# bnbowman/pbccs

Hardware: AMD Instinct MI355X
Metric: CCS ZMWs/sec (and GCUPS) at 1/2/4/8 MI355X vs host-CPU ccs (higher is better)
Workload: dtype f64

## Files before the change

pbccs_amd/csrc/arrow_kernels.hpp:

```cpp
#pragma once

#include <hip/hip_runtime.h>

#include "arrow_device.hpp"

namespace pbccs {

struct ScoreWork {
    int nWork = 0;
    const int* zmw = nullptr;
    const int* nMut = nullptr;
    const long long* mutBase = nullptr;
    const long long* deltaBase = nullptr;
    const long long* waveStart = nullptr;
    const long long* mutStart = nullptr;
    const long long* posStart = nullptr;
    const int* codes = nullptr;
    double* delta = nullptr;
    int* edgeList = nullptr;
    int* edgeCount = nullptr;
    int edgeCap = 0;
    int readLo = 0;
    int readHi = 1 << 30;
    const long long* sel = nullptr;
    const long long* selBase = nullptr;
    const int* nSel = nullptr;
    const double* dev = nullptr;
    int* amb = nullptr;
};

constexpr int kCkptMaxK = 32;
constexpr unsigned long long kCkptBadGeometry = 1ull << 62;
struct CkptWork {
    const int2* pairs = nullptr;
    const long long* taskStart = nullptr;
    int nPairs = 0;
    long long nTasks = 0;
    unsigned long long* counter = nullptr;
    double* slots = nullptr;
    long long slotCap = 0;
    int nSlots = 0;
    unsigned long long* need = nullptr;
};

struct ScoreScratch {
    double* pool = nullptr;
    unsigned long long* top = nullptr;
    unsigned long long cap = 0;
    int* overflow = nullptr;
};

struct FillScratch {
    double* val = nullptr;
    int2* range = nullptr;
    int* off = nullptr;
    double* ls = nullptr;
    double* pre = nullptr;
    int* usedA = nullptr;
    int* usedB = nullptr;
    long long capSlots = 0;
    int capCols = 0;
    long long* trace = nullptr;
};

struct CoopFill {
    int* usedA = nullptr;
    int* usedB = nullptr;
    int* maxH = nullptr;
    int hcap = 0;
    int readWords = 0;
    int tplWords = 0;
    size_t groupBytes = 0;
    bool prio = false;
    bool chainExit = true;
    bool scan = false;
    double devScale = 1.0;
    int rows = 1;
    double thrMargin = 0x1p-50;
    int regrowSlackDiv = 16;
    unsigned long long* valBump = nullptr;
    long long valLimit = 0;
    long long* rValA = nullptr;
    long long* rValB = nullptr;
    long long* rValCap = nullptr;
    double* colScratch = nullptr;
    int gRows = 0;
    long long* trace = nullptr;
    unsigned long long* work = nullptr;
};
enum FillWork : int {
    kFillWorkCells = 0, kFillWorkTallAbort, kFillWorkRegrow, kFillWorkOverflow, kFillWorkSteps, kFillWorkIssues,
    kFillWorkReads, kFillWorkPasses, kFillWorkSlots
};
size_t coop_group_bytes(int hcap, int readWords, int tplWords);
constexpr int kNarrowGroupLanes = 16;
constexpr int kTallRowsPerLane = 2;
void launch_fill_coop(int G, const DevBatch& B, const CoopFill& F, const int* reads, int n, hipStream_t s);

void launch_fill(const DevBatch& B, const FillScratch& F, const int* reads, int n, hipStream_t s);
void launch_compact(const DevBatch& B, const FillScratch& F, const int* reads, int n, hipStream_t s);
void launch_suffix(const DevBatch& B, const int* reads, int n, hipStream_t s, bool withPrefix = false);
void launch_enumerate(const DevBatch& B, const int* zmws, int n, const long long* mutBase, const long long* posBase,
                      int* codes, int* posOff, hipStream_t s);
void launch_score(const DevBatch& B, const ScoreWork& W, long long nWaves, const ScoreScratch& scratch, hipStream_t s,
                  const CkptWork* ck = nullptr);
void launch_alive(const DevBatch& B, const ScoreWork& W, long long nMut, double fastThr, int readHi,
                  unsigned char* alive, hipStream_t s);
void launch_sel_ranges(const ScoreWork& W, const long long* sel, const long long* count, long long* selBase,
                       int* nSel, hipStream_t s);
void launch_reduce(const DevBatch& B, const ScoreWork& W, long long nMut, double fastThr, double* score,
                   unsigned char* fav, hipStream_t s);
void launch_best_subset(int nWork, const long long* selBase, const int* nSel, const int* code, const double* score,
                        int sep, int ldsCap, int* rank, hipStream_t s);
void launch_qv(const DevBatch& B, const ScoreWork& W, long long nPos, const long long* posBase, const int* posOff,
               const double* score, const long long* qvBase, int* qv, hipStream_t s);

}
```

pbccs_amd/csrc/engine.hip:

```cpp
#include "engine.hpp"

#include <hipcub/hipcub.hpp>

#include <algorithm>
#include <mutex>
#include <climits>
#include <cmath>
#include <cstdio>
#include <cstdlib>
#include <cstring>
#include <numeric>
#include <stdexcept>
#include <chrono>
#include <unordered_set>

namespace pbccs {

#define PBCCS_HIP(x)                                                         \
    do {                                                                     \
        hipError_t e_ = (x);                                                 \
        if (e_ != hipSuccess) throw DeviceError(hipGetErrorString(e_));      \
    } while (0)

const char* const kKernelNames[kKernelKinds] = {"k_fill",       "k_suffix",      "k_enumerate", "k_score",
                                                 "k_reduce",     "k_qv",          "k_best_subset", "k_compact",
                                                 "k_fill_tall",  "k_qfill_grp",   "k_qfill_coop", "k_qfill",
                                                 "k_qscore_mid", "k_qscore_multi"};

namespace {

constexpr int kFillBandHeight = 28;
constexpr double kFillScratchBudget = 24.0 * (1ull << 30);
constexpr int kCoopNarrowRows = 64;
constexpr int kCoopTallRows = 1024;
constexpr size_t kCoopLdsBytes = 60 * 1024;
constexpr int kHybridRows = 1536;
constexpr size_t kHeadroomMargin = 24ull << 30;
constexpr long long kTallFirstDiv = 25;
constexpr int kCkptDefaultK = 8;
constexpr int kCkptDefaultMinLen = 4000;
constexpr int kCkptSlotsMax = 2048;
constexpr long long kCkptSlotBytes = 1ll << 30;
int env_int(const char* name, int dflt)
{
    const char* e = std::getenv(name);
    return e ? std::atoi(e) : dflt;
}
constexpr long long kPhasedMinTasks = 1 << 21;
constexpr size_t kInitialScratch = 1 << 20;
constexpr int kMaxCopySegs = 8;

template <class T>
void upload(DevVec<T>& d, const std::vector<T>& h, hipStream_t s)
{
    d.reserve(std::max<size_t>(h.size(), 1), false);
    if (!h.empty()) PBCCS_HIP(hipMemcpyAsync(d.ptr, h.data(), h.size() * sizeof(T), hipMemcpyHostToDevice, s));
}

void d2h(void* dst, const void* src, size_t bytes, hipStream_t s)
{
    static const bool drain = env_int("PBCCS_D2H_DRAIN", 1) != 0;
    if (!bytes) return;
    if (drain) PBCCS_HIP(hipStreamSynchronize(s));
    PBCCS_HIP(hipMemcpyAsync(dst, src, bytes, hipMemcpyDeviceToHost, s));
}

template <class T>
void download(std::vector<T>& h, const DevVec<T>& d, size_t n, hipStream_t s)
{
    h.resize(n);
    d2h(h.data(), d.ptr, n * sizeof(T), s);
}

struct CopySeg {
    const unsigned int* src;
    unsigned int* dst;
    unsigned long long words;
};
struct CopySegs {
    CopySeg s[kMaxCopySegs];
};
__global__ void __launch_bounds__(256) k_copy_segs(CopySegs g)
{
    const CopySeg q = g.s[blockIdx.y];
    for (unsigned long long k = (unsigned long long)blockIdx.x * 256 + threadIdx.x; k < q.words;
         k += (unsigned long long)gridDim.x * 256)
        q.dst[k] = q.src[k];
}

struct Xfer {
    void* dev;
    void* host;
    size_t bytes;
};

size_t stage_layout(const std::vector<Xfer>& items, std::vector<size_t>* off)
{
    size_t top = 0;
    off->clear();
    for (const Xfer& x : items) {
        if (x.bytes % 4) throw DeviceError("packed transfer of a size not a multiple of 4 bytes");
        off->push_back(top);
        top += (x.bytes + 15) & ~(size_t)15;
    }
    return top;
}

void launch_copy_segs(const std::vector<CopySeg>& segs, hipStream_t s)
{
    for (size_t b = 0; b < segs.size(); b += kMaxCopySegs) {
        CopySegs g{};
        const int n = (int)std::min(segs.size() - b, (size_t)kMaxCopySegs);
        unsigned long long most = 0;
        for (int k = 0; k < n; ++k) {
            g.s[k] = segs[b + k];
            most = std::max(most, segs[b + k].words);
        }
        if (!most) continue;
        const unsigned gx = (unsigned)std::min<unsigned long long>((most + 255) / 256, 1024);
        hipLaunchKernelGGL(k_copy_segs, dim3(gx, n), dim3(256), 0, s, g);
        PBCCS_HIP(hipGetLastError());
    }
}

void download_packed(const std::vector<Xfer>& items, DevVec<unsigned char>& stage, std::vector<unsigned char>& host,
                     hipStream_t s)
{
    std::vector<size_t> off;
    const size_t top = stage_layout(items, &off);
    if (!top) return;
    stage.reserve(top, false);
    std::vector<CopySeg> segs;
    for (size_t k = 0; k < items.size(); ++k)
        if (items[k].bytes)
            segs.push_back({static_cast<const unsigned int*>(items[k].dev),
                            reinterpret_cast<unsigned int*>(stage.ptr + off[k]), items[k].bytes / 4});
    launch_copy_segs(segs, s);
    host.resize(top);
    d2h(host.data(), stage.ptr, top, s);
    PBCCS_HIP(hipStreamSynchronize(s));
    for (size_t k = 0; k < items.size(); ++k)
        if (items[k].bytes) std::memcpy(items[k].host, host.data() + off[k], items[k].bytes);
}

void upload_packed(const std::vector<Xfer>& items, DevVec<unsigned char>& stage, std::vector<unsigned char>& host,
                   hipStream_t s)
{
    std::vector<size_t> off;
    const size_t top = stage_layout(items, &off);
    if (!top) return;
    stage.reserve(top, false);
    host.resize(top);
    std::vector<CopySeg> segs;
    for (size_t k = 0; k < items.size(); ++k) {
        if (!items[k].bytes) continue;
        std::memcpy(host.data() + off[k], items[k].host, items[k].bytes);
        segs.push_back({reinterpret_cast<const unsigned int*>(stage.ptr + off[k]),
                        static_cast<unsigned int*>(items[k].dev), items[k].bytes / 4});
    }
    PBCCS_HIP(hipMemcpyAsync(stage.ptr, host.data(), top, hipMemcpyHostToDevice, s));
    launch_copy_segs(segs, s);
}

template <class T>
Xfer xfer_dl(std::vector<T>& h, const DevVec<T>& d, size_t n)
{
    h.resize(n);
    return Xfer{d.ptr, h.data(), n * sizeof(T)};
}

template <class T>
Xfer xfer_ul(DevVec<T>& d, const std::vector<T>& h)
{
    d.reserve(std::max<size_t>(h.size(), 1), false);
    return Xfer{d.ptr, const_cast<T*>(h.data()), h.size() * sizeof(T)};
}

}

static bool va_used_before(void* va)
{
    static std::mutex mu;
    static std::vector<void*> used;
    std::lock_guard<std::mutex> lk(mu);
    if (std::find(used.begin(), used.end(), va) != used.end()) return true;
    used.push_back(va);
    return false;
}

void VmPool::try_reserve(size_t n)
{
    if (!vmm_ || n <= cap) return;
    map_to(n, true);
}

void VmPool::reserve(size_t n, bool keep)
{
    if (n <= cap) return;
    if (!tried_ && allowVmm) {
        tried_ = true;
        void* va = nullptr;
        static const bool dbgVa = env_int("PBCCS_DBG_VA", 0) != 0;
        for (int attempt = 0;; ++attempt) {
            vmm_ = hipMemAddressReserve(&va, kVaBytes, 0, nullptr, 0) == hipSuccess && va != nullptr;
            if (!vmm_) {
                (void)hipGetLastError();
                break;
            }
            if (dbgVa) std::fprintf(stderr, "[vmpool %p] reserve va=%p (%zu parked)\n", (void*)this, va, parkedVas_.size());
            if (!va_used_before(va)) break;
            reusedVas_ += 1;
            parkedVas_.push_back(va);
            if (attempt == 64) throw DeviceError("band pool: no address range this pool has not mapped before");
        }
        if (vmm_) ptr = static_cast<double*>(va);
    }
    if (!vmm_) {
        fallback_.reserve(n, keep);
        ptr = fallback_.ptr;
        cap = fallback_.cap;
        return;
    }
    map_to(n, false);
}

void VmPool::map_to(size_t n, bool soft)
{
    size_t want = n * sizeof(double);
    if (want > kVaBytes) {
        if (!soft) throw DeviceError("band pool exceeds its address reservation");
        want = kVaBytes;
    }
    size_t capBytes = kVaBytes;
    if (const char* e = std::getenv("PBCCS_POOL_CAP_MB")) {
        const long long mb = std::atoll(e);
        if (mb > 0) capBytes = std::min(kVaBytes, (size_t)mb << 20);
    }
    if (want > capBytes) {
        if (!soft)
            throw DeviceOom("band pool capped at " + std::to_string(capBytes >> 20) + " MB (PBCCS_POOL_CAP_MB), needs " +
                            std::to_string(want >> 20) + " MB");
        want = capBytes;
    }
    int dev = 0;
    PBCCS_HIP(hipGetDevice(&dev));
    hipMemAllocationProp prop = {};
    prop.type = hipMemAllocationTypePinned;
    prop.location.type = hipMemLocationTypeDevice;
    prop.location.id = dev;
    hipMemAccessDesc desc = {};
    desc.location = prop.location;
    desc.flags = hipMemAccessFlagsProtReadWrite;
    while (mappedBytes_ < want) {
        const size_t bytes = std::min(std::min(kChunkBytes, capBytes), kVaBytes - mappedBytes_);
        if (mappedBytes_ + bytes > capBytes) break;
        hipMemGenericAllocationHandle_t h;
        if (hipMemCreate(&h, bytes, &prop, 0) != hipSuccess) {
            (void)hipGetLastError();
            if (soft) break;
            size_t fr = 0, tot = 0;
            (void)hipMemGetInfo(&fr, &tot);
            throw DeviceOom("hipMemCreate failed (device memory): band pool at " + std::to_string(mappedBytes_ >> 30) +
                              " GB, needs " + std::to_string(want >> 30) + " GB, " + std::to_string(fr >> 20) +
                              " MB free");
        }
        char* at = reinterpret_cast<char*>(ptr) + mappedBytes_;
        if (hipMemMap(at, bytes, 0, h, 0) != hipSuccess) {
            (void)hipMemRelease(h);
            throw DeviceError("hipMemMap failed");
        }
        if (hipMemSetAccess(at, bytes, &desc, 1) != hipSuccess) {
            (void)hipMemUnmap(at, bytes);
            (void)hipMemRelease(h);
            throw DeviceError("hipMemSetAccess failed");
        }
        handles_.push_back(h);
        sizes_.push_back(bytes);
        mappedBytes_ += bytes;
    }
    cap = mappedBytes_ / sizeof(double);
    if (!soft && mappedBytes_ < want)
        throw DeviceOom("band pool capped at " + std::to_string(capBytes >> 20) + " MB (PBCCS_POOL_CAP_MB), needs " +
                        std::to_string(want >> 20) + " MB");
}

void VmPool::unmap_all(hipStream_t s)
{
    if (!vmm_) {
        if (s) (void)hipStreamSynchronize(s);
        fallback_.release();
        ptr = nullptr;
        cap = 0;
        return;
    }
    if (s) (void)hipStreamSynchronize(s);
    else (void)hipDeviceSynchronize();
    static const bool dbgVa = env_int("PBCCS_DBG_VA", 0) != 0;
    if (dbgVa) std::fprintf(stderr, "[vmpool %p] unmap_all va=%p mapped=%zu MB\n", (void*)this, (void*)ptr, mappedBytes_ >> 20);
    size_t off = 0;
    for (size_t k = 0; k < handles_.size(); ++k) {
        (void)hipMemUnmap(reinterpret_cast<char*>(ptr) + off, sizes_[k]);
        (void)hipMemRelease(handles_[k]);
        off += sizes_[k];
    }
    handles_.clear();
    sizes_.clear();
    mappedBytes_ = 0;
    cap = 0;
    (void)hipMemAddressFree(ptr, kVaBytes);
    ptr = nullptr;
    tried_ = false;
    vmm_ = false;
}

VmPool::~VmPool()
{
    for (void* va : parkedVas_) (void)hipMemAddressFree(va, kVaBytes);
    if (!vmm_) return;
    (void)hipDeviceSynchronize();
    size_t off = 0;
    for (size_t k = 0; k < handles_.size(); ++k) {
        (void)hipMemUnmap(reinterpret_cast<char*>(ptr) + off, sizes_[k]);
        (void)hipMemRelease(handles_[k]);
        off += sizes_[k];
    }
    (void)hipMemAddressFree(ptr, kVaBytes);
}

void ckpt_policy(int* K, int* minLen)
{
    *K = std::min(kCkptMaxK, std::max(0, env_int("PBCCS_CKPT_K", kCkptDefaultK)));
    *minLen = std::max(0, env_int("PBCCS_CKPT_MIN_LEN", kCkptDefaultMinLen));
}

Workspace::~Workspace()
{
    if (stream) (void)hipStreamSynchronize(stream);
    if (stream2) (void)hipStreamSynchronize(stream2);
    for (hipEvent_t e : eventPool) (void)hipEventDestroy(e);
    if (evFork) (void)hipEventDestroy(evFork);
    if (evJoin) (void)hipEventDestroy(evJoin);
    if (stream2) (void)hipStreamDestroy(stream2);
    if (stream) (void)hipStreamDestroy(stream);
}

size_t Workspace::TrimRetired()
{
    size_t b = 0;
    auto t = [&](auto& v) { b += v.trim(); };
    t(hDesc);
    t(selBase); t(nSel); t(colScratch); t(bump); t(desc); t(seq); t(ckPairs); t(ckStart); t(rBaseline); t(rFlips);
    t(rDev); t(wDev); t(wAmb);
    t(rStatus); t(usedA); t(usedB); t(maxH); t(wZmw); t(wNMut); t(wMutBase); t(wDeltaBase); t(wWaveStart);
    t(wMutStart); t(wPosStart); t(wPosBase); t(wQvBase); t(stats); t(aRange); t(bRange); t(aOff); t(bOff); t(aLs);
    t(bLs); t(aPre); t(bSuf); t(fVal); t(fLs); t(fPre); t(fRange); t(fOff); t(codes); t(posOff); t(qv); t(list);
    t(edge); t(edgeCount); t(ckSlots); t(ckCounter); t(delta); t(score); t(fav); t(scratch); t(scratchTop);
    t(scratchOverflow); t(xStage); t(sel); t(selCount); t(selScore); t(selCode); t(selRank); t(selTmp);
    b += val.trim_fallback();
    return b;
}

void Workspace::EnsureStreams()
{
    if (stream) return;
    PBCCS_HIP(hipStreamCreateWithFlags(&stream, hipStreamNonBlocking));
    PBCCS_HIP(hipStreamCreateWithFlags(&stream2, hipStreamNonBlocking));
    PBCCS_HIP(hipEventCreateWithFlags(&evFork, hipEventDisableTiming));
    PBCCS_HIP(hipEventCreateWithFlags(&evJoin, hipEventDisableTiming));
}

ArrowBatch::ArrowBatch(int device, Workspace* shared, bool ownStreams, bool wsBuffers)
    : device_(device),
      ownWs_(shared ? nullptr : new Workspace()),
      ws_(shared ? shared : ownWs_.get()),
      dSelBase_(ws_->selBase), dNSel_(ws_->nSel), dColScratch_(ws_->colScratch), dBump_(ws_->bump),
      hDesc_(ws_->hDesc), dCkPairs_(ws_->ckPairs), dCkStart_(ws_->ckStart), dRBaseline_(ws_->rBaseline),
      dRDev_(ws_->rDev),
      dRFlips_(ws_->rFlips), dRStatus_(ws_->rStatus), dUsedA_(ws_->usedA), dUsedB_(ws_->usedB), dMaxH_(ws_->maxH),
      dWZmw_(ws_->wZmw), dWNMut_(ws_->wNMut), dWMutBase_(ws_->wMutBase), dWDeltaBase_(ws_->wDeltaBase),
      dWWaveStart_(ws_->wWaveStart), dWMutStart_(ws_->wMutStart), dWPosStart_(ws_->wPosStart),
      dWPosBase_(ws_->wPosBase), dWQvBase_(ws_->wQvBase),
      dARange_(ws_->aRange), dBRange_(ws_->bRange), dAOff_(ws_->aOff), dBOff_(ws_->bOff), dALs_(ws_->aLs),
      dBLs_(ws_->bLs), dAPre_(ws_->aPre), dBSuf_(ws_->bSuf), dVal_(ws_->val), dCodes_(ws_->codes),
      dPosOff_(ws_->posOff), dQv_(ws_->qv), dList_(ws_->list), dEdge_(ws_->edge), dEdgeCount_(ws_->edgeCount),
      dDelta_(ws_->delta), dScore_(ws_->score), dFav_(ws_->fav), dScratch_(ws_->scratch),
      dScratchTop_(ws_->scratchTop), dScratchOverflow_(ws_->scratchOverflow), dStats_(ws_->stats),
      eventPool_(ws_->eventPool), dDesc_(wsBuffers && shared ? ws_->desc : ownDesc_),
      dSeq_(wsBuffers && shared ? ws_->seq : ownSeq_)
{
    PBCCS_HIP(hipSetDevice(device_));
    if (const char* e = std::getenv("PBCCS_INITIAL_BAND_HEIGHT")) initialBandHeight_ = std::max(1, std::atoi(e));
    ckpt_policy(&ckptK_, &ckptMinLen_);
    ckptAll_ = std::min(kCkptMaxK, std::max(0, env_int("PBCCS_CKPT_ALL", 0)));
    if (ownStreams) {
        ownStreams_ = true;
        PBCCS_HIP(hipStreamCreateWithFlags(&stream_, hipStreamNonBlocking));
        static const bool oneStream = env_int("PBCCS_ONE_STREAM", 0) != 0;
        if (oneStream) stream2_ = stream_;
        else PBCCS_HIP(hipStreamCreateWithFlags(&stream2_, hipStreamNonBlocking));
        PBCCS_HIP(hipEventCreateWithFlags(&evFork_, hipEventDisableTiming));
        PBCCS_HIP(hipEventCreateWithFlags(&evJoin_, hipEventDisableTiming));
    } else {
        ws_->EnsureStreams();
        stream_ = ws_->stream;
        stream2_ = ws_->stream2;
        evFork_ = ws_->evFork;
        evJoin_ = ws_->evJoin;
    }
    const StreamScope bound(stream_);
    if (shared && std::getenv("PBCCS_DBG_CLEAR") && std::getenv("PBCCS_DBG_CLEAR")[0] == '1') {
        PBCCS_HIP(hipDeviceSynchronize());
        auto z = [](auto& v) {
            if (v.ptr) PBCCS_HIP(hipMemset(v.ptr, 0, v.cap * sizeof(*v.ptr)));
        };
        Workspace& w = *ws_;
        z(w.selBase); z(w.nSel); z(w.colScratch); z(w.bump); z(w.ckPairs); z(w.ckStart); z(w.rBaseline);
        z(w.rFlips); z(w.rStatus); z(w.usedA); z(w.usedB); z(w.maxH); z(w.wZmw); z(w.wNMut); z(w.wMutBase);
        z(w.wDeltaBase); z(w.wWaveStart); z(w.wMutStart); z(w.wPosStart); z(w.wPosBase); z(w.wQvBase); z(w.stats);
        if (w.hDesc.ptr) std::memset(w.hDesc.ptr, 0, w.hDesc.cap);
        PBCCS_HIP(hipDeviceSynchronize());
    }
    dScratch_.reserve(kInitialScratch, false);
    dScratchTop_.reserve(1, false);
    hSeq_.assign(16, '\0');
    seqTop_ = 16;
    dScratchOverflow_.reserve(1, false);
}

ArrowBatch::~ArrowBatch()
{
    if (stream_) {
        (void)hipStreamSynchronize(stream_);
        (void)hipStreamSynchronize(stream2_);
        for (const Pending& p : pending_) {
            eventPool_.push_back(p.a);
            eventPool_.push_back(p.b);
        }
        if (ownStreams_) {
            (void)hipEventDestroy(evFork_);
            (void)hipEventDestroy(evJoin_);
            if (stream2_ != stream_) (void)hipStreamDestroy(stream2_);
            (void)hipStreamDestroy(stream_);
        }
    }
}

void ArrowBatch::SetProfiling(bool on)
{
    const StreamScope bound(stream_);
    profiling_ = on;
    if (on) {
        dStats_.reserve(16, false);
        PBCCS_HIP(hipMemsetAsync(dStats_.ptr, 0, 16 * sizeof(unsigned long long), stream_));
    }
}

template <class F>
void ArrowBatch::Timed(KernelKind k, F&& launch, hipStream_t st)
{
    if (!st) st = stream_;
    static const bool dbgSync = std::getenv("PBCCS_DBG_SYNC") && std::getenv("PBCCS_DBG_SYNC")[0] == '1';
    if (!profiling_) {
        launch();
        if (dbgSync) {
            PBCCS_HIP(hipStreamSynchronize(stream_));
            PBCCS_HIP(hipStreamSynchronize(stream2_));
        }
        return;
    }
    hipEvent_t ev[2];
    for (int i = 0; i < 2; ++i) {
        if (!eventPool_.empty()) {
            ev[i] = eventPool_.back();
            eventPool_.pop_back();
        } else {
            PBCCS_HIP(hipEventCreate(&ev[i]));
        }
    }
    PBCCS_HIP(hipEventRecord(ev[0], st));
    launch();
    PBCCS_HIP(hipEventRecord(ev[1], st));
    pending_.push_back({(int)k, ev[0], ev[1]});
    stats_[k].launches += 1;
}

void ArrowBatch::ResolveEvents()
{
    if (pending_.empty()) return;
    PBCCS_HIP(hipStreamSynchronize(stream_));
    PBCCS_HIP(hipStreamSynchronize(stream2_));
    for (const Pending& p : pending_) {
        float ms = 0.0f;
        if (hipEventElapsedTime(&ms, p.a, p.b) == hipSuccess) stats_[p.kind].ms += ms;
        else (void)hipGetLastError();
        eventPool_.push_back(p.a);
        eventPool_.push_back(p.b);
    }
    pending_.clear();
}

const Counters& ArrowBatch::counters()
{
    const StreamScope bound(stream_);
    if (dFillWork_.ptr) {
        unsigned long long h[16];
        d2h(h, dFillWork_.ptr, sizeof(h), stream_);
        PBCCS_HIP(hipMemsetAsync(dFillWork_.ptr, 0, sizeof(h), stream_));
        PBCCS_HIP(hipStreamSynchronize(stream_));
        for (int k = 0; k < 16; ++k) counters_.fillWork[k] += (long long)h[k];
    }
    long long region = 0, used = 0;
    for (const HRead& r : reads_) {
        region += 2 * r.valCap;
        used += r.usedA + r.usedB;
    }
    counters_.bandTopBytes = std::max(counters_.bandTopBytes, valTop_ * (long long)sizeof(double));
    counters_.bandRegionBytes = std::max(counters_.bandRegionBytes, region * (long long)sizeof(double));
    counters_.bandUsedBytes = std::max(counters_.bandUsedBytes, used * (long long)sizeof(double));
    return counters_;
}

void ArrowBatch::CollectProfile(KernelStat out[kKernelKinds])
{
    const StreamScope bound(stream_);
    ResolveEvents();
    if (profiling_) {
        unsigned long long h[16];
        d2h(h, dStats_.ptr, sizeof(h), stream_);
        PBCCS_HIP(hipStreamSynchronize(stream_));
        stats_[kKFill].cells += (double)h[2 * kStatFill];
        stats_[kKFill].bytes += (double)h[2 * kStatFill + 1];
        stats_[kKFillTall].cells += (double)h[2 * kStatFillTall];
        stats_[kKFillTall].bytes += (double)h[2 * kStatFillTall + 1];
        stats_[kKScore].cells += (double)h[2 * kStatScore];
        stats_[kKScore].bytes += (double)h[2 * kStatScore + 1];
        stats_[kKFill].waveTicks += (double)h[kWaveFill];
        stats_[kKFillTall].waveTicks += (double)h[kWaveFillTall];
        stats_[kKScore].waveTicks += (double)h[kWaveScore];
        stats_[kKSuffix].waveTicks += (double)h[kWaveSuffix];
        stats_[kKReduce].waveTicks += (double)h[kWaveReduce];
        static const bool trace = std::getenv("PBCCS_ROUND_TRACE") != nullptr;
        if (trace) std::fprintf(stderr, "[fillcells] g16=%llu g64=%llu\n", h[8], h[9]);
        PBCCS_HIP(hipMemsetAsync(dStats_.ptr, 0, sizeof(h), stream_));
    }
    for (int k = 0; k < kKernelKinds; ++k) {
        out[k].launches += stats_[k].launches;
        out[k].ms += stats_[k].ms;
        out[k].cells += stats_[k].cells;
        out[k].bytes += stats_[k].bytes;
        out[k].waveTicks += stats_[k].waveTicks;
        stats_[k] = KernelStat();
    }
}

void ArrowBatch::Prepare()
{
    const StreamScope bound(stream_);
    const size_t cols = std::max<long long>(colTop_, 1);
    dARange_.reserve(cols, false);
    dBRange_.reserve(cols, false);
    dAOff_.reserve(cols, false);
    dBOff_.reserve(cols, false);
    dALs_.reserve(cols, false);
    dBLs_.reserve(cols, false);
    dAPre_.reserve(cols, false);
    dBSuf_.reserve(cols, false);
    dVal_.reserve(std::max<long long>(valTop_, 1), false);
    UploadReads();
    long long mut = 0, delta = 0, pos = 0;
    for (const HZmw& z : zmws_) {
        const long long M = unique_mutation_count(z.tpl) + 64;
        mut += M;
        delta += M * z.nReads;
        pos += (long long)z.tpl.size() + 65;
    }
    dCodes_.reserve(std::max<long long>(mut, 1), false);
    dScore_.reserve(std::max<long long>(mut, 1), false);
    dFav_.reserve(std::max<long long>(mut, 1), false);
    dDelta_.reserve(std::max<long long>(delta, 1), false);
    dPosOff_.reserve(std::max<long long>(pos, 1), false);
    dQv_.reserve(std::max<long long>(pos, 1), false);
    ws_->sel.reserve(std::max<long long>(mut, 1), false);
    ws_->selScore.reserve(std::max<long long>(mut, 1), false);
    ws_->selCode.reserve(std::max<long long>(mut, 1), false);
    ws_->selRank.reserve(std::max<long long>(mut, 1), false);
    ws_->selCount.reserve(2, false);
    {
        size_t a = 0, b = 0, c = 0;
        const int nm = (int)std::min<long long>(std::max<long long>(mut, 1), INT_MAX);
        hipcub::CountingInputIterator<long long> it(0);
        PBCCS_HIP(hipcub::DeviceSelect::Flagged(nullptr, a, it, dFav_.ptr, ws_->sel.ptr, ws_->selCount.ptr, nm, stream_));
        PBCCS_HIP(hipcub::DeviceSelect::Flagged(nullptr, b, dScore_.ptr, dFav_.ptr, ws_->selScore.ptr,
                                                ws_->selCount.ptr + 1, nm, stream_));
        PBCCS_HIP(hipcub::DeviceSelect::Flagged(nullptr, c, dCodes_.ptr, dFav_.ptr, ws_->selCode.ptr,
                                                ws_->selCount.ptr + 1, nm, stream_));
        ws_->selTmp.reserve(std::max<size_t>(std::max(a, std::max(b, c)), 1), false);
    }
    PBCCS_HIP(hipStreamSynchronize(stream_));
}

int ArrowBatch::AddZmw(const std::string& tpl, const double snr[4], const ArrowOptions& opt)
{
    if (tpl.empty() || !is_acgt(tpl)) throw std::invalid_argument("template must be a non-empty ACGT string");
    if (!(opt.scoreDiff >= 0.0)) throw std::invalid_argument("ScoreDiff must be positive!");
    HZmw z;
    z.tpl = tpl;
    for (int k = 0; k < 4; ++k) z.snr[k] = snr[k];
    z.opt = opt;
    z.readBegin = (int)reads_.size();
    z.nReads = 0;
    const int L = (int)tpl.size();
    z.tplCap = L + L / 4 + 64;
    z.tplOff = tplTop_;
    tplTop_ += 2LL * z.tplCap;
    zmws_.push_back(z);
    descDirty_ = true;
    return (int)zmws_.size() - 1;
}

void ArrowBatch::DeriveZmws()
{
    const auto t0 = std::chrono::steady_clock::now();
    bool any = false;
    for (size_t zi = 0; zi < zmws_.size(); ++zi) {
        HZmw& z = zmws_[zi];
        if (z.derived) continue;
        transition_table(z.snr, z.trans);
        device_context_table(z.trans, z.ctx);
        for (int k = 0; k < 9; ++k) {
            const std::pair<double, double> mv = expected_context_ll(k < 8 ? z.trans[k] : TransParams(), kMismatchProbability);
            z.ctxMeanVar[k][0] = mv.first;
            z.ctxMeanVar[k][1] = mv.second;
        }
        z.derived = true;
        UploadTemplate((int)zi);
        any = true;
    }
    if (any)
        counters_.deriveNs += std::chrono::duration_cast<std::chrono::nanoseconds>(std::chrono::steady_clock::now() - t0).count();
}

int ArrowBatch::AppendRead(int z, const std::string& seq, int strand, int ts, int te)
{
    if (z != (int)zmws_.size() - 1) throw std::invalid_argument("reads must be appended to the latest ZMW");
    const int L = (int)zmws_[z].tpl.size();
    if (ts < 0 || te > L || ts > te) throw std::invalid_argument("read window outside the template");
    HRead r;
    r.seq = seq;
    r.strand = strand;
    r.ts = ts;
    r.te = te;
    r.zmw = z;
    r.seqOff = seqTop_;
    seqTop_ += (long long)seq.size() + 1;
    hSeq_.insert(hSeq_.end(), seq.begin(), seq.end());
    hSeq_.push_back('\0');
    const int J = te - ts;
    r.colCap = J + J / 4 + 66;
    r.colBase = colTop_;
    colTop_ += r.colCap;
    r.valCap = (long long)(J + 66) * initialBandHeight_;
    r.valA = valTop_;
    r.valB = valTop_ + r.valCap;
    valTop_ += 2 * r.valCap;
    reads_.push_back(r);
    zmws_[z].nReads += 1;
    descDirty_ = true;
    return (int)reads_.size() - 1;
}

void ArrowBatch::UploadTemplate(int zi)
{
    HZmw& z = zmws_[zi];
    const int L = (int)z.tpl.size();
    if (L > z.tplCap) {
        z.tplCap = L + L / 4 + 64;
        z.tplOff = tplTop_;
        tplTop_ += 2LL * z.tplCap;
        descDirty_ = true;
    }
    if ((long long)hTpl_.size() < tplTop_) hTpl_.resize(tplTop_);
    std::memcpy(&hTpl_[z.tplOff], z.tpl.data(), L);
    const std::string rc = reverse_complement(z.tpl);
    std::memcpy(&hTpl_[z.tplOff + z.tplCap], rc.data(), L);
    descDirty_ = true;
}

void ArrowBatch::EnsureCapacity(int ri)
{
    HRead& r = reads_[ri];
    const int J = r.te - r.ts;
    if (J + 2 > r.colCap) {
        r.colCap = J + J / 4 + 66;
        r.colBase = colTop_;
        colTop_ += r.colCap;
        if ((long long)r.colCap * initialBandHeight_ > r.valCap) {
            r.valCap = (long long)r.colCap * initialBandHeight_;
            r.valA = valTop_;
            r.valB = valTop_ + r.valCap;
            valTop_ += 2 * r.valCap;
        }
        descDirty_ = true;
    }
    if (r.valCap == 0) {
        r.valCap = (long long)r.colCap * initialBandHeight_;
        r.valA = valTop_;
        r.valB = valTop_ + r.valCap;
        valTop_ += 2 * r.valCap;
        descDirty_ = true;
    }
}

void ArrowBatch::Retire(const std::vector<int>& zl)
{
    for (int zi : zl) {
        const HZmw& z = zmws_[zi];
        for (int k = 0; k < z.nReads; ++k) reads_[z.readBegin + k].retired = true;
    }
}

bool ArrowBatch::Relayout(const std::vector<int>& list)
{
    if (!reclaim_ || !ws_->val.allowVmm) return false;
    std::vector<char> in(reads_.size(), 0);
    for (int r : list) in[r] = 1;
    for (size_t r = 0; r < reads_.size(); ++r) {
        const HRead& h = reads_[r];
        if (h.filled && h.active && !h.retired && !in[r]) return false;
    }
    for (HRead& h : reads_) {
        h.valCap = 0;
        h.valA = h.valB = 0;
    }
    valTop_ = 0;
    for (int r : list) {
        HRead& h = reads_[r];
        const long long m = std::max(h.usedA, h.usedB);
        long long cap;
        if (h.filled && m > 0) cap = m + m / 8 + 64;
        else if (h.fillPath == 2 || h.fillPath == 3)
            cap = ((long long)h.seq.size() + 1) * (h.te - h.ts + 1) / kTallFirstDiv / std::max(1, h.ckpt) + 64;
        else cap = (long long)h.colCap * initialBandHeight_;
        h.valCap = cap;
        h.valA = valTop_;
        h.valB = valTop_ + cap;
        valTop_ += 2 * cap;
    }
    for (size_t r = 0; r < reads_.size(); ++r)
        if (!in[r]) reads_[r].usedA = reads_[r].usedB = 0;
    descDirty_ = true;
    counters_.relayouts += 1;
    return true;
}

void ArrowBatch::UploadReads()
{
    dSeq_.reserve(hSeq_.size() + 32, true);
    if (hSeq_.size() > seqUploaded_) {
        PBCCS_HIP(hipMemcpyAsync(dSeq_.ptr + seqUploaded_, hSeq_.data() + seqUploaded_, hSeq_.size() - seqUploaded_,
                                 hipMemcpyHostToDevice, stream_));
        seqUploaded_ = hSeq_.size();
    }
}

void ArrowBatch::UploadDescriptors()
{
    const StreamScope bound(stream_);
    DeriveZmws();
    if (!descDirty_) return;
    const int Z = (int)zmws_.size(), R = (int)reads_.size();
    std::vector<int> zf(Z), zr(Z), zl(Z), zb(Z), zn(Z);
    std::vector<double> zc((size_t)Z * 45);
    for (int i = 0; i < Z; ++i) {
        const HZmw& z = zmws_[i];
        zf[i] = (int)z.tplOff;
        zr[i] = (int)(z.tplOff + z.tplCap);
        zl[i] = (int)z.tpl.size();
        zb[i] = z.readBegin;
        zn[i] = z.nReads;
        std::memcpy(&zc[(size_t)i * 45], z.ctx, sizeof(z.ctx));
    }
    std::vector<long long> so(R), cb(R), va(R), vb(R), vc(R);
    std::vector<int> rl(R), rs(R), rts(R), rte(R), ra(R), rz(R), rck(R);
    for (int i = 0; i < R; ++i) {
        const HRead& r = reads_[i];
        so[i] = r.seqOff;
        cb[i] = r.colBase;
        va[i] = r.valA;
        vb[i] = r.valB;
        vc[i] = r.valCap;
        rl[i] = (int)r.seq.size();
        rs[i] = r.strand;
        rts[i] = r.ts;
        rte[i] = r.te;
        ra[i] = r.active ? 1 : 0;
        rz[i] = r.zmw;
        rck[i] = r.ckpt;
    }
    size_t top = 0;
    auto place = [&](size_t bytes) {
        const size_t at = top;
        top += (bytes + 255) & ~(size_t)255;
        return at;
    };
    const size_t oZf = place(Z * sizeof(int)), oZr = place(Z * sizeof(int)), oZl = place(Z * sizeof(int)),
                 oZb = place(Z * sizeof(int)), oZn = place(Z * sizeof(int)), oZc = place(zc.size() * sizeof(double));
    const size_t oSo = place(R * sizeof(long long)), oCb = place(R * sizeof(long long)),
                 oVa = place(R * sizeof(long long)), oVb = place(R * sizeof(long long)),
                 oVc = place(R * sizeof(long long));
    const size_t oRl = place(R * sizeof(int)), oRs = place(R * sizeof(int)), oRts = place(R * sizeof(int)),
                 oRte = place(R * sizeof(int)), oRa = place(R * sizeof(int)), oRz = place(R * sizeof(int)),
                 oRck = place(R * sizeof(int));
    const size_t oTpl = place(hTpl_.size() + 32);
    hDesc_.reserve(std::max<size_t>(top, 1));
    auto put = [&](size_t at, const void* src, size_t bytes) {
        if (bytes) std::memcpy(hDesc_.ptr + at, src, bytes);
    };
    put(oZf, zf.data(), Z * sizeof(int));
    put(oZr, zr.data(), Z * sizeof(int));
    put(oZl, zl.data(), Z * sizeof(int));
    put(oZb, zb.data(), Z * sizeof(int));
    put(oZn, zn.data(), Z * sizeof(int));
    put(oZc, zc.data(), zc.size() * sizeof(double));
    put(oSo, so.data(), R * sizeof(long long));
    put(oCb, cb.data(), R * sizeof(long long));
    put(oVa, va.data(), R * sizeof(long long));
    put(oVb, vb.data(), R * sizeof(long long));
    put(oVc, vc.data(), R * sizeof(long long));
    put(oRl, rl.data(), R * sizeof(int));
    put(oRs, rs.data(), R * sizeof(int));
    put(oRts, rts.data(), R * sizeof(int));
    put(oRte, rte.data(), R * sizeof(int));
    put(oRa, ra.data(), R * sizeof(int));
    put(oRz, rz.data(), R * sizeof(int));
    put(oRck, rck.data(), R * sizeof(int));
    put(oTpl, hTpl_.data(), hTpl_.size());
    dDesc_.reserve(std::max<size_t>(top, 1), false);
    PBCCS_HIP(hipMemcpyAsync(dDesc_.ptr, hDesc_.ptr, top, hipMemcpyHostToDevice, stream_));
    char* base = dDesc_.ptr;
    pZFwd_ = reinterpret_cast<int*>(base + oZf);
    pZRev_ = reinterpret_cast<int*>(base + oZr);
    pZLen_ = reinterpret_cast<int*>(base + oZl);
    pZReadBegin_ = reinterpret_cast<int*>(base + oZb);
    pZNReads_ = reinterpret_cast<int*>(base + oZn);
    pZCtx_ = reinterpret_cast<double*>(base + oZc);
    pRSeqOff_ = reinterpret_cast<long long*>(base + oSo);
    pRColBase_ = reinterpret_cast<long long*>(base + oCb);
    pRValA_ = reinterpret_cast<long long*>(base + oVa);
    pRValB_ = reinterpret_cast<long long*>(base + oVb);
    pRValCap_ = reinterpret_cast<long long*>(base + oVc);
    pRLen_ = reinterpret_cast<int*>(base + oRl);
    pRStrand_ = reinterpret_cast<int*>(base + oRs);
    pRTs_ = reinterpret_cast<int*>(base + oRts);
    pRTe_ = reinterpret_cast<int*>(base + oRte);
    pRActive_ = reinterpret_cast<int*>(base + oRa);
    pRZmw_ = reinterpret_cast<int*>(base + oRz);
    pRCkpt_ = reinterpret_cast<int*>(base + oRck);
    pTpl_ = base + oTpl;
    UploadReads();
    const size_t cols = std::max<long long>(colTop_, 1);
    dARange_.reserve(cols, true);
    dBRange_.reserve(cols, true);
    dAOff_.reserve(cols, true);
    dBOff_.reserve(cols, true);
    dALs_.reserve(cols, true);
    dBLs_.reserve(cols, true);
    dAPre_.reserve(cols, true);
    dBSuf_.reserve(cols, true);
    dVal_.reserve(std::max<long long>(valTop_, 1), true);
    dRBaseline_.reserve(std::max(R, 1), true);
    dRDev_.reserve(std::max(R, 1), true);
    dRFlips_.reserve(std::max(R, 1), true);
    dRStatus_.reserve(std::max(R, 1), true);
    PBCCS_HIP(hipStreamSynchronize(stream_));
    descDirty_ = false;
}

DevBatch ArrowBatch::View() const
{
    DevBatch b;
    b.zFwdOff = pZFwd_;
    b.zRevOff = pZRev_;
    b.zLen = pZLen_;
    b.zCtx = pZCtx_;
    b.zReadBegin = pZReadBegin_;
    b.zNReads = pZNReads_;
    b.tplPool = pTpl_;
    b.rSeqOff = pRSeqOff_;
    b.rLen = pRLen_;
    b.rStrand = pRStrand_;
    b.rTs = pRTs_;
    b.rTe = pRTe_;
    b.rActive = pRActive_;
    b.rZmw = pRZmw_;
    b.rColBase = pRColBase_;
    b.rValA = pRValA_;
    b.rValB = pRValB_;
    b.rValCap = pRValCap_;
    b.rCkpt = pRCkpt_;
    b.seqPool = dSeq_.ptr;
    b.aRange = dARange_.ptr;
    b.aOff = dAOff_.ptr;
    b.aLs = dALs_.ptr;
    b.aPre = dAPre_.ptr;
    b.bRange = dBRange_.ptr;
    b.bOff = dBOff_.ptr;
    b.bLs = dBLs_.ptr;
    b.bSuf = dBSuf_.ptr;
    b.valPool = dVal_.ptr;
    b.rBaseline = dRBaseline_.ptr;
    b.rDev = dRDev_.ptr;
    b.rFlips = dRFlips_.ptr;
    b.rStatus = dRStatus_.ptr;
    b.prNot = 1.0 - kMismatchProbability;
    b.prThird = kMismatchProbability / 3.0;
    b.sdn = zmws_.empty() ? std::exp(12.5) : std::exp(zmws_[0].opt.scoreDiff);
    b.stats = profiling_ ? dStats_.ptr : nullptr;
    return b;
}

void ArrowBatch::FillReads(const std::vector<int>& readsIn)
{
    const StreamScope bound(stream_);
    constexpr int kPaths = 4;
    for (int r : readsIn) EnsureCapacity(r);
    auto promote = [&](int r, int p) {
        HRead& h = reads_[r];
        int q = p + 1;
        if (q == 2 && (long long)h.seq.size() + 1 > 4LL * kCoopTallRows) q = 3;
        h.fillPath = q;
        if (q >= 2 && q < kPaths) {
            const long long I = (long long)h.seq.size(), J = h.te - h.ts;
            const bool ck = ckptAll_ > 0 || (ckptK_ > 0 && J >= ckptMinLen_);
            const long long K = ck ? std::max(ckptAll_, ckptK_) : 1;
            const long long want = (I + 1) * (J + 1) / kTallFirstDiv / K + (ck ? 2 * (kCkptTail + 1) * (I + 1) : 0) + 64;
            if (want > h.valCap) {
                h.valCap = want;
                h.valA = valTop_;
                h.valB = valTop_ + h.valCap;
                valTop_ += 2 * h.valCap;
                descDirty_ = true;
            }
        }
        return q;
    };
    Relayout(readsIn);
    std::vector<int> todo[kPaths], serial, done;
    for (int r : readsIn) {
        const int p = reads_[r].fillPath;
        if (p >= kPaths) serial.push_back(r);
        else todo[p].push_back(r);
    }
    auto words = [&](int r) {
        return (int)(reads_[r].seq.size() + 7) / 8 + (reads_[r].te - reads_[r].ts + 8) / 8;
    };
    constexpr int tallG = 64;
    static const int tallRows = env_int("PBCCS_TALL_ROWS", kTallRowsPerLane) == 1 ? 1 : 2;
    const long long chunk = (long long)tallG * tallRows;
    const long long tallGroupLds = (long long)kCoopLdsBytes;
    auto full_rows = [&](int maxI) { return ((long long)maxI + chunk) / chunk * chunk; };
    constexpr int narrowG = kNarrowGroupLanes;
    constexpr int narrowRows = 1;
    auto rows_for = [&](int p, int maxI, int w) -> int {
        if (p == 0) return 0;
        if (p == 1)
            return (64 / narrowG) * coop_group_bytes(kCoopNarrowRows, w, 0) <= kCoopLdsBytes
                       ? kCoopNarrowRows : 0;
        const long long room = (tallGroupLds - (long long)coop_group_bytes(0, w, 0)) / 16 / 64 * 64;
        const long long full = full_rows(maxI);
        if (p == 2) {
            const long long want = std::min<long long>(kCoopTallRows, full);
            return room >= want ? (int)want : 0;
        }
        static const long long hybLds = (long long)env_int("PBCCS_HYBRID_LDS_KB", (int)(kCoopLdsBytes >> 10)) << 10;
        static const long long hybRows = env_int("PBCCS_HYBRID_ROWS", kHybridRows);
        const long long hroom = (std::min<long long>(hybLds, 160 << 10) - (long long)coop_group_bytes(0, w, 0)) / 16 / 64 * 64;
        const long long want = std::min(std::min(full, hroom), hybRows);
        return want >= 64 ? (int)want : 0;
    };
    static const bool pathTrace = std::getenv("PBCCS_FILL_PATHS") != nullptr;
    static const bool pathTrace2 = pathTrace && std::getenv("PBCCS_FILL_PATHS")[0] == '2';
    static const bool fillWork = std::getenv("PBCCS_FILL_WORK") != nullptr;
    for (int attempt = 0;; ++attempt) {
        for (int p = 0; p < kPaths; ++p) {
            std::vector<int> keep;
            for (int r : todo[p]) {
                if (rows_for(p, (int)reads_[r].seq.size(), words(r)) > 0) keep.push_back(r);
                else if (p + 1 < kPaths) todo[p + 1].push_back(r);
                else {
                    reads_[r].fillPath = kPaths;
                    serial.push_back(r);
                }
            }
            todo[p].swap(keep);
        }
        if (std::all_of(todo, todo + kPaths, [](const std::vector<int>& v) { return v.empty(); })) break;
        if (attempt > 8) throw DeviceError("band storage keeps overflowing");
        auto quick = [&](int x) { return reads_[x].filled && reads_[x].flips == 0 ? 1 : 0; };
        auto high = [&](int x) {
            const HRead& h = reads_[x];
            return h.filled && std::max(h.usedA, h.usedB) > 16LL * (h.te - h.ts + 1) ? 0 : 1;
        };
        for (int p = 0; p < kPaths; ++p) {
            auto& v = todo[p];
            if (p >= 2) {
                std::stable_sort(v.begin(), v.end(), [&](int x, int y) {
                    return std::max(reads_[x].usedA, reads_[x].usedB) > std::max(reads_[y].usedA, reads_[y].usedB);
                });
                continue;
            }
            std::stable_sort(v.begin(), v.end(), [&](int x, int y) {
                const int qx = quick(x), qy = quick(y);
                if (qx != qy) return qx < qy;
                const int hx = high(x), hy = high(y);
                if (hx != hy) return hx < hy;
                return reads_[x].te - reads_[x].ts > reads_[y].te - reads_[y].ts;
            });
        }
        for (int p = 0; p < kPaths; ++p)
            for (int r : todo[p]) {
                HRead& h = reads_[r];
                int k = 0;
                if (ckptAll_ > 0 && p >= 1) k = ckptAll_;
                else if (ckptK_ > 0 && p >= 2 && h.te - h.ts >= ckptMinLen_) k = ckptK_;
                if (h.ckpt != k) {
                    h.ckpt = k;
                    descDirty_ = true;
                }
            }
        const int scanPaths = env_int("PBCCS_SCAN_PATHS", 1);
        auto scannable = [&](int r) { return scan_ && !reads_[r].exact; };
        int nScan[kPaths] = {};
        for (int p = 2; p < kPaths; ++p) {
            if (!((scanPaths >> (p - 2)) & 1)) continue;
            std::stable_partition(todo[p].begin(), todo[p].end(), scannable);
            nScan[p] = (int)std::count_if(todo[p].begin(), todo[p].end(), scannable);
        }
        const bool anyScan = nScan[2] + nScan[3] > 0;
        UploadDescriptors();
        const size_t R = reads_.size();
        dUsedA_.reserve(std::max<size_t>(R, 1), true);
        dUsedB_.reserve(std::max<size_t>(R, 1), true);
        dMaxH_.reserve(std::max<size_t>(R, 1), true);
        std::vector<int> list;
        for (auto& v : todo) list.insert(list.end(), v.begin(), v.end());
        upload(dList_, list, stream_);
        const DevBatch B = View();
        size_t off = 0;
        const bool forked = !todo[2].empty() || !todo[3].empty();
        const auto tLaunch = std::chrono::steady_clock::now();
        const bool grow = ws_->val.allowVmm;
        long long headroom = 0;
        if (grow) {
            long long want = 1ll << 24;
            for (int p = 2; p < kPaths; ++p)
                for (int r : todo[p]) {
                    const long long I = (long long)reads_[r].seq.size(), J = reads_[r].te - reads_[r].ts;
                    const long long K = std::max(1, reads_[r].ckpt);
                    want += 2 * std::max<long long>(0, (I + 1) * (J + 1) / 7 / K - reads_[r].valCap);
                }
            size_t freeB = 0, totalB = 0;
            PBCCS_HIP(hipMemGetInfo(&freeB, &totalB));
            static const long long margin = (long long)env_int("PBCCS_HEADROOM_MARGIN_GB", (int)(kHeadroomMargin >> 30)) << 30;
            const long long spare = std::max<long long>(0, (long long)freeB - margin);
            headroom = std::min<long long>(want, spare / 4 / (long long)sizeof(double));
            dVal_.reserve((size_t)std::max<long long>(valTop_, 1), true);
            dVal_.try_reserve((size_t)std::max<long long>(valTop_ + headroom, 1));
            dBump_.reserve(1, false);
            const unsigned long long top = (unsigned long long)valTop_;
            PBCCS_HIP(hipMemcpyAsync(dBump_.ptr, &top, sizeof(top), hipMemcpyHostToDevice, stream_));
        }
        const long long valLimit = grow ? (long long)dVal_.cap : 0;
        if (forked) {
            PBCCS_HIP(hipEventRecord(evFork_, stream_));
            PBCCS_HIP(hipStreamWaitEvent(stream2_, evFork_, 0));
        }
        for (int p = 0; p < kPaths; ++p) {
            const int n = (int)todo[p].size();
            if (n == 0) continue;
            int maxI = 1, maxJ = 1;
            for (int r : todo[p]) {
                maxI = std::max(maxI, (int)reads_[r].seq.size());
                maxJ = std::max(maxJ, reads_[r].te - reads_[r].ts);
            }
            CoopFill F;
            F.usedA = dUsedA_.ptr;
            F.usedB = dUsedB_.ptr;
            F.maxH = dMaxH_.ptr;
            F.readWords = (maxI + 7) / 8;
            F.tplWords = (maxJ + 8) / 8;
            F.hcap = rows_for(p, maxI, F.readWords + F.tplWords);
            const int G = p == 1 ? narrowG : tallG;
            F.rows = p == 1 ? narrowRows : tallRows;
            F.prio = p >= 2;
            if (const char* e = std::getenv("PBCCS_FILL_THR_MARGIN"))
                F.thrMargin = std::max(0x1p-50, std::atof(e));
            F.groupBytes = coop_group_bytes(F.hcap, F.readWords, F.tplWords);
            const int full = (int)full_rows(maxI);
            if (p == 3 && full > F.hcap) {
                F.gRows = full - F.hcap;
                dColScratch_.reserve((size_t)n * 2 * F.gRows, false);
                F.colScratch = dColScratch_.ptr;
            }
            if (grow) {
                F.valBump = dBump_.ptr;
                F.valLimit = valLimit;
                F.rValA = pRValA_;
                F.rValB = pRValB_;
                F.rValCap = pRValCap_;
            }
            const int* lp = dList_.ptr + off;
            const hipStream_t st = p <= 1 ? stream_ : stream2_;
            if (fillWork) {
                if (!dFillWork_.ptr) {
                    dFillWork_.reserve(16, false);
                    PBCCS_HIP(hipMemsetAsync(dFillWork_.ptr, 0, 16 * sizeof(unsigned long long), stream_));
                }
                F.work = dFillWork_.ptr;
            }
            if (pathTrace2) {
                dCoopTrace_[p].reserve((size_t)6 * n, false);
                PBCCS_HIP(hipMemsetAsync(dCoopTrace_[p].ptr, 0, sizeof(long long) * 6 * n, st));
                F.trace = dCoopTrace_[p].ptr;
            }
            const int nScan2 = nScan[p];
            if (nScan2 > 0) {
                CoopFill FS = F;
                FS.scan = true;
                if (const char* e = std::getenv("PBCCS_SCAN_DEV_SCALE")) FS.devScale = std::max(1.0, std::atof(e));
                Timed(p == 1 ? kKFill : kKFillTall, [&] { launch_fill_coop(G, B, FS, lp, nScan2, st); }, st);
                PBCCS_HIP(hipGetLastError());
                counters_.fillLaunches += 1;
                counters_.scanReads += nScan2;
                if (n > nScan2) {
                    Timed(p == 1 ? kKFill : kKFillTall, [&] { launch_fill_coop(G, B, F, lp + nScan2, n - nScan2, st); },
                          st);
                    PBCCS_HIP(hipGetLastError());
                    counters_.fillLaunches += 1;
                }
            } else {
                Timed(p == 1 ? kKFill : kKFillTall, [&] { launch_fill_coop(G, B, F, lp, n, st); }, st);
                PBCCS_HIP(hipGetLastError());
                counters_.fillLaunches += 1;
            }
            off += n;
        }
        if (forked) {
            PBCCS_HIP(hipEventRecord(evJoin_, stream2_));
            PBCCS_HIP(hipStreamWaitEvent(stream_, evJoin_, 0));
            static const bool joinSync = std::getenv("PBCCS_DBG_JOINSYNC") && std::getenv("PBCCS_DBG_JOINSYNC")[0] == '1';
            if (joinSync) PBCCS_HIP(hipStreamSynchronize(stream2_));
        }
        std::vector<int> st, fl, ua, ub, mh;
        std::vector<double> bl, dv;
        unsigned long long bump = (unsigned long long)valTop_;
        {
            std::vector<Xfer> xs{xfer_dl(mh, dMaxH_, R), xfer_dl(st, dRStatus_, R), xfer_dl(fl, dRFlips_, R),
                                 xfer_dl(bl, dRBaseline_, R), xfer_dl(ua, dUsedA_, R), xfer_dl(ub, dUsedB_, R)};
            if (anyScan) xs.push_back(xfer_dl(dv, dRDev_, R));
            if (grow) xs.push_back(Xfer{dBump_.ptr, &bump, sizeof(bump)});
            download_packed(xs, ws_->xStage, hXStage_, stream_);
        }
        if (grow && bump != (unsigned long long)valTop_) {
            std::vector<long long> va, vb, vc;
            va.resize(R);
            vb.resize(R);
            vc.resize(R);
            d2h(va.data(), pRValA_, R * sizeof(long long), stream_);
            d2h(vb.data(), pRValB_, R * sizeof(long long), stream_);
            d2h(vc.data(), pRValCap_, R * sizeof(long long), stream_);
            PBCCS_HIP(hipStreamSynchronize(stream_));
            for (auto& v : todo)
                for (int r : v) {
                    reads_[r].valA = va[r];
                    reads_[r].valB = vb[r];
                    reads_[r].valCap = vc[r];
                }
            valTop_ = (long long)std::min<unsigned long long>(bump, (unsigned long long)valLimit);
            counters_.bandGrowths += 1;
        }
        if (pathTrace) {
            int nt = 0, no = 0;
            for (int p = 0; p < kPaths; ++p)
                for (int r : todo[p]) {
                    nt += st[r] == kFillTall;
                    no += st[r] == kFillOverflow;
                }
            std::fprintf(stderr, "[fillpaths] batch=%p attempt=%d n=%zu/%zu/%zu/%zu wall=%.1fms tall=%d ovf=%d\n",
                         (void*)this, attempt, todo[0].size(), todo[1].size(), todo[2].size(), todo[3].size(),
                         std::chrono::duration<double, std::milli>(std::chrono::steady_clock::now() - tLaunch).count(),
                         nt, no);
            for (int p = 1; pathTrace2 && p < kPaths; ++p) {
                const size_t n = todo[p].size();
                if (n == 0) continue;
                std::vector<long long> tr;
                download(tr, dCoopTrace_[p], 6 * n, stream_);
                PBCCS_HIP(hipStreamSynchronize(stream_));
                long long t0 = LLONG_MAX, t1 = 0;
                size_t slow = 0;
                double sumCells = 0, sumCyc = 0;
                for (size_t t = 0; t < n; ++t) {
                    if (tr[6 * t + 1] <= 0) continue;
                    t0 = std::min(t0, tr[6 * t]);
                    t1 = std::max(t1, tr[6 * t + 1]);
                    if (tr[6 * t + 1] - tr[6 * t] > tr[6 * slow + 1] - tr[6 * slow]) slow = t;
                    sumCells += (double)tr[6 * t + 3];
                    sumCyc += (double)tr[6 * t + 2];
                }
                const long long* s = &tr[6 * slow];
                std::fprintf(stderr, "[fillread] path=%d n=%zu span=%.1fms slowest: %.1fms %.1f cyc/cell cells=%lld "
                             "passes=%lld cols=%lld; all: %.1f cyc/cell\n", p, n, (t1 - t0) / 1e5, (s[1] - s[0]) / 1e5,
                             s[3] ? (double)s[2] / (double)s[3] : 0.0, s[3], s[4], s[5],
                             sumCells > 0 ? sumCyc / sumCells : 0.0);
            }
        }
        std::vector<int> next[kPaths];
        for (int p = 0; p < kPaths; ++p) {
            for (int r : todo[p]) {
                HRead& h = reads_[r];
                if (st[r] == kFillTall) {
                    const int q = promote(r, p);
                    if (q >= kPaths) serial.push_back(r);
                    else next[q].push_back(r);
                    continue;
                }
                if (st[r] == kFillUncertain) {
                    h.exact = true;
                    counters_.uncertainReads += 1;
                    for (int bit = 0; bit < 4; ++bit) counters_.uncertainWhy[bit] += (fl[r] >> bit) & 1;
                    next[p].push_back(r);
                    continue;
                }
                if (st[r] == kFillOverflow) {
                    const long long need = std::max(ua[r], ub[r]);
                    h.valCap = std::max(need + need / 16 + 64, h.valCap + 1);
                    h.valA = valTop_;
                    h.valB = valTop_ + h.valCap;
                    valTop_ += 2 * h.valCap;
                    descDirty_ = true;
                    next[p].push_back(r);
                    continue;
                }
                h.status = st[r];
                h.flips = fl[r];
                h.baseline = bl[r];
                h.dev = !dv.empty() ? dv[r] : 0.0;
                h.filled = true;
                h.usedA = ua[r];
                h.usedB = ub[r];
                if (p >= 1) h.maxH = mh[r];
                if (st[r] == kFillOk || st[r] == kFillMismatch) done.push_back(r);
            }
        }
        for (int p = 0; p < kPaths; ++p) todo[p].swap(next[p]);
    }
    if (!done.empty()) {
        upload(dList_, done, stream_);
        const DevBatch B = View();
        Timed(kKSuffix, [&] { launch_suffix(B, dList_.ptr, (int)done.size(), stream_, true); });
        PBCCS_HIP(hipGetLastError());
        PBCCS_HIP(hipStreamSynchronize(stream_));
    }
    if (!serial.empty()) FillReadsSerial(serial);
    (void)counters();
}

void ArrowBatch::FillReadsSerial(const std::vector<int>& readsIn)
{
    const StreamScope bound(stream_);
    std::vector<int> todo(readsIn);
    for (int r : todo)
        if (reads_[r].ckpt != 0) {
            reads_[r].ckpt = 0;
            descDirty_ = true;
        }
    for (int r : todo) EnsureCapacity(r);
    int H = kFillBandHeight;
    for (int attempt = 0; !todo.empty(); ++attempt) {
        if (attempt > 8) throw DeviceError("band storage keeps overflowing");
        std::stable_sort(todo.begin(), todo.end(), [&](int x, int y) {
            return reads_[x].te - reads_[x].ts > reads_[y].te - reads_[y].ts;
        });
        UploadDescriptors();
        const size_t R = reads_.size();
        dUsedA_.reserve(std::max<size_t>(R, 1), true);
        dUsedB_.reserve(std::max<size_t>(R, 1), true);
        std::vector<int> again;
        size_t pos = 0;
        while (pos < todo.size()) {
            const int capCols = reads_[todo[pos]].te - reads_[todo[pos]].ts + 2;
            const long long capSlots = (long long)capCols * H + 64;
            const double perGroup = 2.0 * capSlots * 64 * 8 + 2.0 * capCols * 64 * 20 + (capCols + 1.0) * 64 * 8;
            const long long maxGroups = std::max<long long>(1, (long long)(kFillScratchBudget / perGroup));
            const size_t n = std::min<size_t>(todo.size() - pos, (size_t)maxGroups * 64);
            std::vector<int> chunk(todo.begin() + pos, todo.begin() + pos + n);
            const long long groups = (long long)(n + 63) / 64;
            ws_->fVal.reserve((size_t)(2 * groups * capSlots * 64), false);
            ws_->fRange.reserve((size_t)(2 * groups * capCols * 64), false);
            ws_->fOff.reserve((size_t)(2 * groups * capCols * 64), false);
            ws_->fLs.reserve((size_t)(2 * groups * capCols * 64), false);
            ws_->fPre.reserve((size_t)(groups * (capCols + 1) * 64), false);
            FillScratch F;
            F.val = ws_->fVal.ptr;
            F.range = ws_->fRange.ptr;
            F.off = ws_->fOff.ptr;
            F.ls = ws_->fLs.ptr;
            F.pre = ws_->fPre.ptr;
            F.usedA = dUsedA_.ptr;
            F.usedB = dUsedB_.ptr;
            F.capSlots = capSlots;
            F.capCols = capCols;
            static const bool trace = std::getenv("PBCCS_FILL_TRACE") != nullptr;
            if (trace) {
                dTrace_.reserve(8 * n, false);
                F.trace = dTrace_.ptr;
            }
            upload(dList_, chunk, stream_);
            const DevBatch B = View();
            Timed(kKFillTall, [&] { launch_fill(B, F, dList_.ptr, (int)n, stream_); });
            PBCCS_HIP(hipGetLastError());
            counters_.fillLaunches += 1;
            std::vector<int> st, fl, ua, ub;
            std::vector<double> bl;
            download_packed({xfer_dl(st, dRStatus_, R), xfer_dl(fl, dRFlips_, R), xfer_dl(bl, dRBaseline_, R),
                             xfer_dl(ua, dUsedA_, R), xfer_dl(ub, dUsedB_, R)},
                            ws_->xStage, hXStage_, stream_);
            if (trace) TraceSummary(n, H, capSlots);
            for (int r : chunk) {
                HRead& h = reads_[r];
                if (st[r] == kFillOverflow) {
                    again.push_back(r);
                    continue;
                }
                h.status = st[r];
                h.flips = fl[r];
                h.baseline = bl[r];
                h.dev = 0.0;
                h.filled = true;
                h.usedA = ua[r];
                h.usedB = ub[r];
                if (st[r] == kFillOk || st[r] == kFillMismatch) {
                    const long long need = std::max(ua[r], ub[r]);
                    if (need > h.valCap) {
                        h.valCap = need + need / 4 + 64;
                        h.valA = valTop_;
                        h.valB = valTop_ + h.valCap;
                        valTop_ += 2 * h.valCap;
                        descDirty_ = true;
                    }
                }
            }
            UploadDescriptors();
            const DevBatch B2 = View();
            Timed(kKCompact, [&] { launch_compact(B2, F, dList_.ptr, (int)n, stream_); });
            Timed(kKSuffix, [&] { launch_suffix(B2, dList_.ptr, (int)n, stream_); });
            PBCCS_HIP(hipGetLastError());
            PBCCS_HIP(hipStreamSynchronize(stream_));
            pos += n;
        }
        todo.swap(again);
        H *= 2;
    }
}

void ArrowBatch::TraceSummary(size_t n, int H, long long capSlots)
{
    std::vector<long long> tr;
    download(tr, dTrace_, 8 * n, stream_);
    PBCCS_HIP(hipStreamSynchronize(stream_));
    long long t0 = LLONG_MAX, t1 = 0, maxDur = 0, maxCells = 0, sumCells = 0, sumPass = 0, maxPass = 0;
    double sumDur = 0;
    long long done = 0;
    for (size_t t = 0; t < n; ++t) {
        const long long* e = &tr[8 * t];
        if (e[1] <= 0) continue;
        ++done;
        t0 = std::min(t0, e[0]);
        t1 = std::max(t1, e[1]);
        maxDur = std::max(maxDur, e[1] - e[0]);
        sumDur += double(e[1] - e[0]);
        maxCells = std::max(maxCells, e[2]);
        sumCells += e[2];
        sumPass += e[3];
        maxPass = std::max(maxPass, e[3]);
    }
    std::fprintf(stderr,
                 "[fill-trace] lanes=%zu done=%lld H=%d capSlots=%lld span_ms=%.3f maxlane_ms=%.3f avglane_ms=%.3f "
                 "cells avg=%.0f max=%lld passes avg=%.2f max=%lld\n",
                 n, done, H, capSlots, (t1 - t0) / 1e5, maxDur / 1e5, done ? sumDur / done / 1e5 : 0.0,
                 done ? double(sumCells) / done : 0.0, maxCells, done ? double(sumPass) / done : 0.0, maxPass);
}

void ArrowBatch::MeanVar(const HZmw& z, int strand, int ts, int te, double* mean, double* var) const
{
    const std::string t = strand == kFwd ? z.tpl : reverse_complement(z.tpl);
    const int L = (int)t.size();
    double m = 0.0, v = 0.0;
    for (int i = ts; i < te - 1; ++i) {
        const int c = (i + 1 < L) ? context_index(t[i], t[i + 1]) : kCtxZero;
        m += z.ctxMeanVar[c][0];
        v += z.ctxMeanVar[c][1];
    }
    *mean = m;
    *var = v;
}

void ArrowBatch::CertifyAddReads(const std::vector<int>& readsIn, double threshold)
{
    if (std::isnan(threshold)) return;
    std::vector<int> redo;
    for (int ri : readsIn) {
        HRead& r = reads_[ri];
        if (r.dev <= 0.0 || r.status != kFillOk || !std::isfinite(r.baseline)) continue;
        double mean = 0.0, var = 0.0;
        MeanVar(zmws_[r.zmw], r.strand, r.ts, r.te, &mean, &var);
        const double sd = std::sqrt(var);
        const double z = (r.baseline - mean) / sd;
        if (!std::isfinite(z) || std::fabs(z - threshold) <= (r.dev + 4.0 * kUnitRoundoff * (std::fabs(r.baseline) +
                                                                                          std::fabs(mean))) / sd +
                                                                  8.0 * kUnitRoundoff * std::fabs(z)) {
            r.exact = true;
            redo.push_back(ri);
        }
    }
    if (redo.empty()) return;
    counters_.uncertainReads += (long long)redo.size();
    FillReads(redo);
}

int ArrowBatch::FinishAddRead(int ri, double threshold)
{
    HRead& r = reads_[ri];
    int res = kSuccess;
    if (r.status == kFillBadInput) res = kOther;
    else if (r.status == kFillMismatch || std::isinf(r.baseline)) res = kAlphaBetaMismatch;
    if (res == kSuccess && !std::isnan(threshold)) {
        double mean = 0.0, var = 0.0;
        MeanVar(zmws_[r.zmw], r.strand, r.ts, r.te, &mean, &var);
        const double ll = r.baseline;
        const double z = (ll - mean) / std::sqrt(var);
        if (!std::isfinite(ll) || !std::isfinite(z) || z < threshold) res = kPoorZScore;
    }
    r.active = res == kSuccess;
    descDirty_ = true;
    return res;
}

double ArrowBatch::BaselineScore(int zi) const
{
    const HZmw& z = zmws_[zi];
    double s = 0.0;
    for (int k = 0; k < z.nReads; ++k) {
        const HRead& r = reads_[z.readBegin + k];
        if (r.active) s += r.baseline;
    }
    return s;
}

void ArrowBatch::ZScores(int zi, double* zg, double* za, std::vector<double>* zs) const
{
    const HZmw& z = zmws_[zi];
    const double nan = std::numeric_limits<double>::quiet_NaN();
    zs->clear();
    double gmean = 0.0, gvar = 0.0;
    size_t n = 0;
    for (int k = 0; k < z.nReads; ++k) {
        const HRead& r = reads_[z.readBegin + k];
        if (!r.active) { zs->push_back(nan); continue; }
        n += 1;
        const int s = r.ts, e = r.te - 1;
        if (e - s < 1) { zs->push_back(nan); continue; }
        double mu = 0.0, var = 0.0;
        MeanVar(z, r.strand, r.ts, r.te, &mu, &var);
        gmean += mu;
        gvar += var;
        zs->push_back((r.baseline - mu) / std::sqrt(var));
    }
    const double gs = BaselineScore(zi);
    *zg = (gvar == 0.0) ? nan : (gs - gmean) / std::sqrt(gvar);
    *za = (n == 0 || gvar == 0.0) ? nan : (gs / n - gmean / n) / std::sqrt(gvar / n);
}

void ArrowBatch::RunRound(const std::vector<int>& zl, const std::vector<std::vector<int>>* codes, double fastThr,
                          bool needPositions, bool phased)
{
    const StreamScope bound(stream_);
    UploadDescriptors();
    const int n = (int)zl.size();
    rNMut_.assign(n, 0);
    rMutStart_.assign(n + 1, 0);
    rPosStart_.assign(n + 1, 0);
    rDeltaBase_.assign(n, 0);
    std::vector<long long> waveStart(n + 1, 0), posBase(n, 0);
    long long delta = 0, posOffTotal = 0;
    for (int k = 0; k < n; ++k) {
        const HZmw& z = zmws_[zl[k]];
        const long long M = codes ? (long long)(*codes)[k].size() : unique_mutation_count(z.tpl);
        rNMut_[k] = (int)M;
        rMutStart_[k + 1] = rMutStart_[k] + M;
        rDeltaBase_[k] = delta;
        delta += M * z.nReads;
        waveStart[k + 1] = waveStart[k] + (long long)z.nReads * ((M + 63) / 64);
        rPosStart_[k + 1] = rPosStart_[k] + (long long)z.tpl.size();
        posBase[k] = posOffTotal;
        posOffTotal += (long long)z.tpl.size() + 1;
    }
    rTotalMut_ = rMutStart_[n];
    rTotalPos_ = rPosStart_[n];
    rTotalDelta_ = delta;
    std::vector<long long> mutBase(rMutStart_.begin(), rMutStart_.begin() + n);
    upload_packed({xfer_ul(dWZmw_, zl), xfer_ul(dWNMut_, rNMut_), xfer_ul(dWMutBase_, mutBase),
                   xfer_ul(dWDeltaBase_, rDeltaBase_), xfer_ul(dWWaveStart_, waveStart), xfer_ul(dWMutStart_, rMutStart_),
                   xfer_ul(dWPosStart_, rPosStart_), xfer_ul(dWPosBase_, posBase)},
                  ws_->xStage, hXStage_, stream_);
    dCodes_.reserve(std::max<long long>(rTotalMut_, 1), false);
    dScore_.reserve(std::max<long long>(rTotalMut_, 1), false);
    dFav_.reserve(std::max<long long>(rTotalMut_, 1), false);
    dDelta_.reserve(std::max<long long>(rTotalDelta_, 1), false);
    const DevBatch B = View();
    if (codes) {
        std::vector<int> flat;
        flat.reserve(rTotalMut_);
        for (const std::vector<int>& c : *codes) flat.insert(flat.end(), c.begin(), c.end());
        upload(dCodes_, flat, stream_);
        PBCCS_HIP(hipStreamSynchronize(stream_));
    } else {
        dPosOff_.reserve(std::max<long long>(posOffTotal, 1), false);
        Timed(kKEnumerate, [&] {
            launch_enumerate(B, dWZmw_.ptr, n, dWMutBase_.ptr, dWPosBase_.ptr, dCodes_.ptr, dPosOff_.ptr, stream_);
        });
    }
    (void)needPositions;
    ScoreWork W;
    W.nWork = n;
    W.zmw = dWZmw_.ptr;
    W.nMut = dWNMut_.ptr;
    W.mutBase = dWMutBase_.ptr;
    W.deltaBase = dWDeltaBase_.ptr;
    W.waveStart = dWWaveStart_.ptr;
    W.mutStart = dWMutStart_.ptr;
    W.posStart = dWPosStart_.ptr;
    W.codes = dCodes_.ptr;
    W.delta = dDelta_.ptr;
    {
        std::vector<double> dev(n, 0.0);
        bool any = false;
        for (int k = 0; k < n; ++k) {
            const HZmw& z = zmws_[zl[k]];
            for (int q = 0; q < z.nReads; ++q) {
                const HRead& h = reads_[z.readBegin + q];
                if (h.active && h.dev > 0.0) dev[k] += 3.0 * h.dev;
            }
            any = any || dev[k] > 0.0;
        }
        rDevItem_ = dev;
        if (any) {
            upload(ws_->wDev, dev, stream_);
            ws_->wAmb.reserve(std::max(n, 1), false);
            PBCCS_HIP(hipMemsetAsync(ws_->wAmb.ptr, 0, std::max(n, 1) * sizeof(int), stream_));
            W.dev = ws_->wDev.ptr;
            W.amb = ws_->wAmb.ptr;
        }
        rAmbOn_ = any;
    }
    long long edgeCap = 0;
    for (int k = 0; k < n; ++k) edgeCap += 80LL * zmws_[zl[k]].nReads;
    edgeCap = std::min<long long>(std::max<long long>(edgeCap, 64), rTotalDelta_ + 64);
    dEdge_.reserve(3 * edgeCap, false);
    dEdgeCount_.reserve(1, false);
    W.edgeList = dEdge_.ptr;
    W.edgeCount = dEdgeCount_.ptr;
    W.edgeCap = (int)edgeCap;
    bool anyCkpt = false;
    for (int k = 0; k < n && !anyCkpt; ++k) {
        const HZmw& z = zmws_[zl[k]];
        for (int q = 0; q < z.nReads; ++q) anyCkpt = anyCkpt || reads_[z.readBegin + q].ckpt != 0;
    }
    CkptWork ck;
    auto ckpt_tasks = [&](int lo, int hi, const std::vector<int>* nSelH) {
        ck = CkptWork();
        if (!anyCkpt) return;
        std::vector<int2> pairs;
        std::vector<long long> start{0};
        long long maxI = 1;
        int maxK = 1;
        for (int k = 0; k < n; ++k) {
            const HZmw& z = zmws_[zl[k]];
            const long long mc = nSelH ? (*nSelH)[k] : rNMut_[k];
            if (mc <= 0) continue;
            for (int q = std::max(0, lo); q < std::min(hi, z.nReads); ++q) {
                const HRead& h = reads_[z.readBegin + q];
                if (h.ckpt == 0) continue;
                pairs.push_back(make_int2(k, q));
                start.push_back(start.back() + (mc + 63) / 64);
                maxI = std::max<long long>(maxI, (long long)h.seq.size() + 1);
                maxK = std::max(maxK, h.ckpt);
            }
        }
        if (pairs.empty()) return;
        upload(dCkPairs_, pairs, stream_);
        upload(dCkStart_, start, stream_);
        ws_->ckCounter.reserve(2, false);
        const long long first = (3LL * maxK + 4) * std::min<long long>(maxI, 1024);
        ckSlotCap_ = std::max(ckSlotCap_, first);
        ck.pairs = dCkPairs_.ptr;
        ck.taskStart = dCkStart_.ptr;
        ck.nPairs = (int)pairs.size();
        ck.nTasks = start.back();
        ck.counter = ws_->ckCounter.ptr;
        ck.need = ws_->ckCounter.ptr + 1;
        ck.nSlots = (int)std::min<long long>(ck.nTasks, kCkptSlotsMax);
    };
    ckpt_tasks(0, 1 << 30, nullptr);
    auto score_launch = [&](long long nWaves) {
        for (int attempt = 0;; ++attempt) {
            PBCCS_HIP(hipMemsetAsync(dEdgeCount_.ptr, 0, sizeof(int), stream_));
            PBCCS_HIP(hipMemsetAsync(dScratchTop_.ptr, 0, sizeof(unsigned long long), stream_));
            PBCCS_HIP(hipMemsetAsync(dScratchOverflow_.ptr, 0, sizeof(int), stream_));
            ScoreScratch sc;
            sc.pool = dScratch_.ptr;
            sc.top = dScratchTop_.ptr;
            sc.cap = dScratch_.cap;
            sc.overflow = dScratchOverflow_.ptr;
            if (ck.nTasks > 0) {
                const long long fit = kCkptSlotBytes / std::max<long long>(1, ckSlotCap_ * (long long)sizeof(double));
                ck.nSlots = (int)std::max<long long>(
                    1, std::min<long long>(std::min<long long>(ck.nTasks, kCkptSlotsMax), std::max<long long>(64, fit)));
                ws_->ckSlots.reserve((size_t)ck.nSlots * ckSlotCap_, false);
                ck.slots = ws_->ckSlots.ptr;
                ck.slotCap = ckSlotCap_;
                PBCCS_HIP(hipMemsetAsync(ws_->ckCounter.ptr, 0, 2 * sizeof(unsigned long long), stream_));
            }
            Timed(kKScore, [&] { launch_score(B, W, nWaves, sc, stream_, ck.nTasks > 0 ? &ck : nullptr); });
            PBCCS_HIP(hipGetLastError());
            int ovf = 0;
            unsigned long long ckNeed = 0;
            d2h(&ovf, dScratchOverflow_.ptr, sizeof(int), stream_);
            if (ck.nTasks > 0)
                d2h(&ckNeed, ck.need, sizeof(ckNeed), stream_);
            PBCCS_HIP(hipStreamSynchronize(stream_));
            if (ckNeed >= kCkptBadGeometry) throw DeviceError("checkpoint replay: block outgrew its column tables");
            if (ckNeed > 0) {
                if (attempt > 8) throw DeviceError("checkpoint replay slots keep overflowing");
                ckSlotCap_ = (long long)ckNeed + (long long)ckNeed / 4 + 64;
                continue;
            }
            if (!ovf) break;
            if (attempt > 8) throw DeviceError("scratch overflow");
            if (ovf & 1) dScratch_.reserve(dScratch_.cap * 4, false);
            if (ovf & 2) {
                edgeCap *= 4;
                dEdge_.reserve(3 * edgeCap, false);
                W.edgeList = dEdge_.ptr;
                W.edgeCap = (int)std::min<long long>(edgeCap, INT_MAX / 4);
            }
        }
    };
    const char* minEnv = std::getenv("PBCCS_PHASED_MIN_TASKS");
    const long long minTasks = minEnv ? std::atoll(minEnv) : kPhasedMinTasks;
    long long tasks = rTotalDelta_;
    if (phased && minTasks >= 0 && rTotalDelta_ >= minTasks && rTotalMut_ <= INT_MAX) {
        static const std::vector<int> bounds = [] {
            std::vector<int> b{0};
            const char* e = std::getenv("PBCCS_PHASE_BOUNDS");
            std::string spec = e ? e : "3,5";
            size_t pos = 0;
            while (pos < spec.size()) {
                const size_t c = spec.find(',', pos);
                const int v = std::atoi(spec.substr(pos, c == std::string::npos ? std::string::npos : c - pos).c_str());
                if (v > b.back()) b.push_back(v);
                if (c == std::string::npos) break;
                pos = c + 1;
            }
            b.push_back(1 << 30);
            return b;
        }();
        const int nPhases = (int)bounds.size() - 1;
        std::vector<std::vector<long long>> ws(nPhases);
        std::vector<int> nSel;
        ws_->sel.reserve(std::max<long long>(rTotalMut_, 1), false);
        ws_->selCount.reserve(2, false);
        dSelBase_.reserve(std::max(n, 1), false);
        dNSel_.reserve(std::max(n, 1), false);
        tasks = 0;
        for (int ph = 0; ph < nPhases; ++ph) {
            const int lo = bounds[ph], hi = bounds[ph + 1];
            if (ph > 0) {
                Timed(kKReduce, [&] { launch_alive(B, W, rTotalMut_, fastThr, lo, dFav_.ptr, stream_); });
                size_t tb = 0;
                hipcub::CountingInputIterator<long long> it(0);
                PBCCS_HIP(hipcub::DeviceSelect::Flagged(nullptr, tb, it, dFav_.ptr, ws_->sel.ptr, ws_->selCount.ptr,
                                                        (int)rTotalMut_, stream_));
                ws_->selTmp.reserve(std::max<size_t>(tb, 1), false);
                PBCCS_HIP(hipcub::DeviceSelect::Flagged(ws_->selTmp.ptr, tb, it, dFav_.ptr, ws_->sel.ptr,
                                                        ws_->selCount.ptr, (int)rTotalMut_, stream_));
                launch_sel_ranges(W, ws_->sel.ptr, ws_->selCount.ptr, dSelBase_.ptr, dNSel_.ptr, stream_);
                PBCCS_HIP(hipGetLastError());
                download(nSel, dNSel_, n, stream_);
                PBCCS_HIP(hipStreamSynchronize(stream_));
                W.sel = ws_->sel.ptr;
                W.selBase = dSelBase_.ptr;
                W.nSel = dNSel_.ptr;
            }
            std::vector<long long>& wsv = ws[ph];
            wsv.assign(n + 1, 0);
            for (int k = 0; k < n; ++k) {
                const int nr = zmws_[zl[k]].nReads;
                const long long reads = std::max(0, std::min(hi, nr) - lo);
                const long long mc = ph == 0 ? rNMut_[k] : nSel[k];
                wsv[k + 1] = wsv[k] + reads * ((mc + 63) / 64);
                tasks += reads * mc;
            }
            if (wsv[n] == 0) break;
            W.readLo = lo;
            W.readHi = hi;
            upload(dWWaveStart_, wsv, stream_);
            W.waveStart = dWWaveStart_.ptr;
            ckpt_tasks(lo, hi, ph == 0 ? nullptr : &nSel);
            score_launch(wsv[n]);
        }
        W.sel = nullptr;
        W.selBase = nullptr;
        W.nSel = nullptr;
        W.readLo = 0;
        W.readHi = 1 << 30;
    } else {
        score_launch(waveStart[n]);
    }
    Timed(kKReduce, [&] { launch_reduce(B, W, rTotalMut_, fastThr, dScore_.ptr, dFav_.ptr, stream_); });
    PBCCS_HIP(hipGetLastError());
    counters_.scoreLaunches += 1;
    counters_.scoreTasks += tasks;
    counters_.mutations += rTotalMut_;
}

void ArrowBatch::ScoreLists(const std::vector<int>& zl, const std::vector<std::vector<int>>& codes, double fastThr,
                            std::vector<std::vector<double>>* scores, std::vector<std::vector<double>>* perRead)
{
    const StreamScope bound(stream_);
    RunRound(zl, &codes, fastThr, false);
    std::vector<double> s, d;
    download(s, dScore_, rTotalMut_, stream_);
    if (perRead) download(d, dDelta_, rTotalDelta_, stream_);
    PBCCS_HIP(hipStreamSynchronize(stream_));
    scores->assign(zl.size(), {});
    if (perRead) perRead->assign(zl.size(), {});
    for (size_t k = 0; k < zl.size(); ++k) {
        (*scores)[k].assign(s.begin() + rMutStart_[k], s.begin() + rMutStart_[k + 1]);
        if (perRead) {
            const int nr = zmws_[zl[k]].nReads;
            (*perRead)[k].assign(d.begin() + rDeltaBase_[k], d.begin() + rDeltaBase_[k] + (long long)nr * rNMut_[k]);
        }
    }
}

static bool apply_host(std::string* tpl, const std::vector<Mutation>& muts, std::vector<int>* mtp)
{
    std::string next;
    if (!apply_mutations(*tpl, muts, &next, mtp)) return false;
    *tpl = next;
    return true;
}

bool ArrowBatch::ApplyMutations(int zi, const std::vector<Mutation>& muts)
{
    const StreamScope bound(stream_);
    HZmw& z = zmws_[zi];
    std::vector<int> mtp;
    if (!apply_host(&z.tpl, muts, &mtp)) return false;
    UploadTemplate(zi);
    std::vector<int> refill;
    for (int k = 0; k < z.nReads; ++k) {
        HRead& r = reads_[z.readBegin + k];
        r.ts = mtp[r.ts];
        r.te = mtp[r.te];
        if (r.active) refill.push_back(z.readBegin + k);
    }
    descDirty_ = true;
    FillReads(refill);
    for (int r : refill)
        if (reads_[r].status != kFillOk) reads_[r].active = false;
    descDirty_ = true;
    return true;
}

namespace {

struct Scored {
    int code;
    float score;
};

std::vector<Scored> best_subset(std::vector<Scored> in, int sep)
{
    if (sep == 0) return in;
    std::vector<Scored> out;
    while (!in.empty()) {
        size_t best = 0;
        for (size_t k = 1; k < in.size(); ++k)
            if (in[best].score < in[k].score) best = k;
        const Scored b = in[best];
        out.push_back(b);
        const int lo = mut_pos(b.code) - sep, hi = mut_pos(b.code) + sep;
        std::vector<Scored> keep;
        keep.reserve(in.size());
        for (const Scored& s : in)
            if (!(lo <= mut_pos(s.code) && mut_pos(s.code) <= hi)) keep.push_back(s);
        in.swap(keep);
    }
    return out;
}

bool best_subset_certain(const std::vector<Scored>& in, const std::vector<double>& sc, double e, int sep)
{
    const size_t n = in.size();
    if (n == 0 || e <= 0.0) return true;
    std::vector<float> lo(n), hi(n);
    for (size_t i = 0; i < n; ++i) {
        const double w = e + 4.0 * kUnitRoundoff * std::fabs(sc[i]);
        lo[i] = (float)(sc[i] - w);
        hi[i] = (float)(sc[i] + w);
    }
    std::vector<char> alive(n, 1);
    for (;;) {
        size_t best = n;
        for (size_t k = 0; k < n; ++k)
            if (alive[k] && (best == n || in[best].score < in[k].score)) best = k;
        if (best == n) return true;
        for (size_t k = 0; k < n; ++k) {
            if (!alive[k] || k == best) continue;
            if (hi[k] < lo[best]) continue;
            const bool fixedTie = lo[k] == hi[k] && lo[best] == hi[best] && lo[k] == lo[best] && k > best;
            if (!fixedTie) return false;
        }
        const int bp = mut_pos(in[best].code);
        if (sep == 0) {
            alive[best] = 0;
            continue;
        }
        for (size_t k = 0; k < n; ++k)
            if (alive[k] && bp - sep <= mut_pos(in[k].code) && mut_pos(in[k].code) <= bp + sep) alive[k] = 0;
    }
}

}

void ArrowBatch::Refine(const std::vector<int>& zl, const RefineOptions& ro, std::vector<int>* converged,
                        std::vector<long long>* nTested, std::vector<long long>* nApplied, bool needFinalState,
                        std::vector<std::vector<int>>* qvsOnConverge)
{
    const StreamScope bound(stream_);
    const int n = (int)zl.size();
    converged->assign(n, 0);
    if (qvsOnConverge) qvsOnConverge->assign(n, {});
    const bool retireDone = reclaim_ && !needFinalState;
    nTested->assign(n, 0);
    nApplied->assign(n, 0);
    std::vector<char> done(n, 0);
    std::vector<std::unordered_set<std::string>> history(n);
    std::vector<std::vector<int>> centers(n);
    std::vector<int> zit(n, 0);
    struct Memo {
        int anchor = 0;
        std::string rtpl;
        std::vector<int> rwin;
        std::vector<int> rcen;
        std::vector<Scored> fav;
        bool same(const Memo& o) const { return rtpl == o.rtpl && rwin == o.rwin && rcen == o.rcen; }
    };
    std::vector<std::vector<Memo>> memo(n);
    static const bool noReplay = std::getenv("PBCCS_NO_CYCLE_REPLAY") != nullptr;
    constexpr int kMaxPeriod = 4;
    auto make_memo = [&](int k) {
        const HZmw& z = zmws_[zl[k]];
        Memo m;
        int a = (int)z.tpl.size();
        for (int q = 0; q < z.nReads; ++q) a = std::min(a, reads_[z.readBegin + q].ts);
        m.anchor = a;
        m.rtpl = z.tpl.substr(std::max(0, a - 1));
        for (int q = 0; q < z.nReads; ++q) {
            const HRead& r = reads_[z.readBegin + q];
            m.rwin.push_back(r.ts - a);
            m.rwin.push_back(r.te - a);
            m.rwin.push_back(r.active ? 1 : 0);
        }
        for (int c : centers[k]) m.rcen.push_back(c - a);
        return m;
    };
    auto match = [&](int k, const Memo& cur) -> int {
        const int i = zit[k];
        for (int p = 1; p <= kMaxPeriod && p <= i; ++p)
            if (cur.same(memo[k][i - p])) return p;
        return 0;
    };
    const double fastThr = zl.empty() ? -12.5 : zmws_[zl[0]].opt.fastScoreThreshold;
    static const bool roundTrace = std::getenv("PBCCS_ROUND_TRACE") != nullptr;
    if (roundTrace)
        std::fprintf(stderr, "[round] batch=%p start zmws=%d bandtop=%.2fGB\n", (void*)this, n, valTop_ * 8.0 / 1e9);
    using Clock = std::chrono::steady_clock;
    auto ms = [](Clock::time_point a, Clock::time_point b) {
        return std::chrono::duration<double, std::milli>(b - a).count();
    };
    std::vector<int> finalRefill;
    long long replayed = 0;
    for (int round = 0;; ++round) {
        const Clock::time_point t0 = Clock::now();
        std::vector<int> preRefill;
        for (int k = 0; k < n; ++k) {
            if (done[k]) continue;
            Memo cur = make_memo(k);
            int p = (noReplay || zit[k] == 0) ? 0 : match(k, cur);
            if (p == 0) {
                memo[k].push_back(std::move(cur));
                continue;
            }
            HZmw& z = zmws_[zl[k]];
            bool ended = false;
            while (p > 0) {
                const int i = zit[k];
                memo[k].push_back(std::move(cur));
                const int shift = memo[k][i].anchor - memo[k][i - p].anchor;
                std::vector<Scored> fav;
                for (const Scored& f : memo[k][i - p].fav)
                    fav.push_back({mut_code(mut_pos(f.code) + shift, mut_type(f.code), mut_base(f.code)), f.score});
                memo[k][i].fav = fav;
                std::vector<char> succActive(z.nReads);
                for (int q = 0; q < z.nReads; ++q) succActive[q] = memo[k][i - p + 1].rwin[3 * q + 2] != 0;
                std::vector<int> tried;
                nearby_mutations(z.tpl, centers[k], ro.mutationNeighborhood, &tried);
                (*nTested)[k] += (long long)tried.size();
                std::vector<Scored> best = best_subset(fav, ro.mutationSeparation);
                std::vector<Mutation> muts;
                for (const Scored& b : best) muts.push_back(mutation_from_code(b.code));
                if (best.size() > 1) {
                    std::string next;
                    std::vector<int> mtp;
                    if (apply_mutations(z.tpl, muts, &next, &mtp) && history[k].count(next)) {
                        best.resize(1);
                        muts.resize(1);
                    }
                }
                (*nApplied)[k] += (long long)best.size();
                history[k].insert(z.tpl);
                centers[k].clear();
                for (const Scored& f : fav) centers[k].push_back(mut_pos(f.code));
                std::vector<int> mtp;
                if (!apply_host(&z.tpl, muts, &mtp)) {
                    done[k] = 1;
                    converged->at(k) = -1;
                    ended = true;
                    break;
                }
                for (int q = 0; q < z.nReads; ++q) {
                    HRead& r = reads_[z.readBegin + q];
                    r.ts = mtp[r.ts];
                    r.te = mtp[r.te];
                    r.active = succActive[q] != 0;
                }
                ++replayed;
                if (++zit[k] >= ro.maxIterations) {
                    done[k] = 1;
                    ended = true;
                    break;
                }
                cur = make_memo(k);
                p = match(k, cur);
            }
            UploadTemplate(zl[k]);
            descDirty_ = true;
            if (!ended) memo[k].push_back(std::move(cur));
            std::vector<int>& dst = ended ? finalRefill : preRefill;
            if (ended && !needFinalState) {
                if (retireDone) Retire({zl[k]});
                continue;
            }
            for (int q = 0; q < z.nReads; ++q)
                if (reads_[z.readBegin + q].active) {
                    EnsureCapacity(z.readBegin + q);
                    dst.push_back(z.readBegin + q);
                }
        }
        if (!preRefill.empty()) {
            FillReads(preRefill);
            for (int r : preRefill)
                if (reads_[r].status != kFillOk) reads_[r].active = false;
            descDirty_ = true;
        }
        std::vector<int> act, idx;
        for (int k = 0; k < n; ++k)
            if (!done[k]) { act.push_back(zl[k]); idx.push_back(k); }
        if (act.empty()) break;
        std::vector<std::vector<int>> lists;
        if (round == 0) {
            RunRound(act, nullptr, fastThr, false, true);
        } else {
            lists.resize(act.size());
            for (size_t a = 0; a < act.size(); ++a)
                nearby_mutations(zmws_[act[a]].tpl, centers[idx[a]], ro.mutationNeighborhood, &lists[a]);
            RunRound(act, &lists, fastThr, false, true);
        }
        for (size_t a = 0; a < act.size(); ++a) (*nTested)[idx[a]] += rNMut_[a];
        const Clock::time_point t1 = Clock::now();

        auto select_round = [&](const std::vector<int>& actL, std::vector<std::vector<Scored>>& favL,
                                std::vector<std::vector<std::pair<int, Scored>>>& pickedL,
                                std::vector<std::vector<double>>& favD) {
            DevVec<long long>& dSel = ws_->sel;
            DevVec<double>& dSelScore = ws_->selScore;
            DevVec<long long>& dCount = ws_->selCount;
            dSel.reserve(std::max<long long>(rTotalMut_, 1), false);
            dSelScore.reserve(std::max<long long>(rTotalMut_, 1), false);
            dCount.reserve(2, false);
            size_t tmpBytes = 0, tmpBytes2 = 0;
            hipcub::CountingInputIterator<long long> it(0);
            PBCCS_HIP(hipcub::DeviceSelect::Flagged(nullptr, tmpBytes, it, dFav_.ptr, dSel.ptr, dCount.ptr,
                                                    (int)rTotalMut_, stream_));
            PBCCS_HIP(hipcub::DeviceSelect::Flagged(nullptr, tmpBytes2, dScore_.ptr, dFav_.ptr, dSelScore.ptr,
                                                    dCount.ptr + 1, (int)rTotalMut_, stream_));
            DevVec<unsigned char>& tmp = ws_->selTmp;
            tmp.reserve(std::max<size_t>(std::max(tmpBytes, tmpBytes2), 1), false);
            PBCCS_HIP(hipcub::DeviceSelect::Flagged(tmp.ptr, tmpBytes, it, dFav_.ptr, dSel.ptr, dCount.ptr,
                                                    (int)rTotalMut_, stream_));
            PBCCS_HIP(hipcub::DeviceSelect::Flagged(tmp.ptr, tmpBytes2, dScore_.ptr, dFav_.ptr, dSelScore.ptr,
                                                    dCount.ptr + 1, (int)rTotalMut_, stream_));
            DevVec<int>& dSelCode = ws_->selCode;
            dSelCode.reserve(std::max<long long>(rTotalMut_, 1), false);
            size_t tb = 0;
            PBCCS_HIP(hipcub::DeviceSelect::Flagged(nullptr, tb, dCodes_.ptr, dFav_.ptr, dSelCode.ptr, dCount.ptr + 1,
                                                    (int)rTotalMut_, stream_));
            tmp.reserve(std::max<size_t>(tb, 1), false);
            PBCCS_HIP(hipcub::DeviceSelect::Flagged(tmp.ptr, tb, dCodes_.ptr, dFav_.ptr, dSelCode.ptr, dCount.ptr + 1,
                                                    (int)rTotalMut_, stream_));
            const int nAct = (int)actL.size();
            dSelBase_.reserve(std::max(nAct, 1), false);
            dNSel_.reserve(std::max(nAct, 1), false);
            DevVec<int>& dSelRank = ws_->selRank;
            dSelRank.reserve(std::max<long long>(rTotalMut_, 1), false);
            ScoreWork SW;
            SW.nWork = nAct;
            SW.mutStart = dWMutStart_.ptr;
            launch_sel_ranges(SW, dSel.ptr, dCount.ptr, dSelBase_.ptr, dNSel_.ptr, stream_);
            const char* capEnv = std::getenv("PBCCS_BEST_LDS");
            Timed(kKSelect, [&] {
                launch_best_subset(nAct, dSelBase_.ptr, dNSel_.ptr, dSelCode.ptr, dSelScore.ptr, ro.mutationSeparation,
                                   capEnv ? std::atoi(capEnv) : -1, dSelRank.ptr, stream_);
            });
            PBCCS_HIP(hipGetLastError());
            long long cnt[2] = {0, 0};
            d2h(cnt, dCount.ptr, 2 * sizeof(long long), stream_);
            PBCCS_HIP(hipStreamSynchronize(stream_));
            std::vector<long long> sel;
            std::vector<double> selScore;
            std::vector<int> selCode, selRank;
            download_packed({xfer_dl(sel, dSel, cnt[0]), xfer_dl(selScore, dSelScore, cnt[0]),
                             xfer_dl(selCode, dSelCode, cnt[0]), xfer_dl(selRank, dSelRank, cnt[0])},
                            ws_->xStage, hXStage_, stream_);

            favL.assign(actL.size(), {});
            pickedL.assign(actL.size(), {});
            favD.assign(actL.size(), {});
            for (size_t q = 0; q < sel.size(); ++q) {
                const long long g = sel[q];
                const size_t a = std::upper_bound(rMutStart_.begin(), rMutStart_.end(), g) - rMutStart_.begin() - 1;
                const Scored e{selCode[q], (float)selScore[q]};
                favL[a].push_back(e);
                favD[a].push_back(selScore[q]);
                if (selRank[q] > 0) pickedL[a].emplace_back(selRank[q], e);
            }
        };
        std::vector<std::vector<Scored>> fav;
        std::vector<std::vector<std::pair<int, Scored>>> picked;
        std::vector<std::vector<double>> favD;
        select_round(act, fav, picked, favD);
        if (rAmbOn_) {
            std::vector<int> ambFlag;
            download(ambFlag, ws_->wAmb, act.size(), stream_);
            PBCCS_HIP(hipStreamSynchronize(stream_));
            std::vector<int> redo;
            for (size_t a = 0; a < act.size(); ++a) {
                const double e = rDevItem_[a];
                if (e <= 0.0) continue;
                if (ambFlag[a] || !best_subset_certain(fav[a], favD[a], e, ro.mutationSeparation)) redo.push_back((int)a);
            }
            if (!redo.empty()) {
                std::vector<int> actR, readsR;
                std::vector<std::vector<int>> listsR;
                for (int a : redo) {
                    actR.push_back(act[a]);
                    if (round > 0) listsR.push_back(lists[a]);
                    const HZmw& z = zmws_[act[a]];
                    for (int q = 0; q < z.nReads; ++q) {
                        HRead& h = reads_[z.readBegin + q];
                        h.exact = true;
                        if (h.active) readsR.push_back(z.readBegin + q);
                    }
                }
                counters_.exactRounds += (long long)redo.size();
                FillReads(readsR);
                for (int r : readsR)
                    if (reads_[r].status != kFillOk) reads_[r].active = false;
                descDirty_ = true;
                RunRound(actR, round == 0 ? nullptr : &listsR, fastThr, false, true);
                std::vector<std::vector<Scored>> favR;
                std::vector<std::vector<std::pair<int, Scored>>> pickedR;
                std::vector<std::vector<double>> favDR;
                select_round(actR, favR, pickedR, favDR);
                for (size_t i = 0; i < redo.size(); ++i) {
                    fav[redo[i]] = std::move(favR[i]);
                    picked[redo[i]] = std::move(pickedR[i]);
                }
            }
        }
        const bool checkBest = std::getenv("PBCCS_CHECK_BEST_SUBSET") != nullptr;
        std::vector<int> changed, qvNow, qvIdx;
        for (size_t a = 0; a < act.size(); ++a) {
            const int k = idx[a];
            const int zi = act[a];
            memo[k].back().fav = fav[a];
            if (fav[a].empty()) {
                converged->at(k) = 1;
                done[k] = 1;
                if (qvsOnConverge) {
                    qvNow.push_back(zi);
                    qvIdx.push_back(k);
                }
                continue;
            }
            std::sort(picked[a].begin(), picked[a].end(),
                      [](const std::pair<int, Scored>& x, const std::pair<int, Scored>& y) { return x.first < y.first; });
            std::vector<Scored> best;
            for (const std::pair<int, Scored>& p : picked[a]) best.push_back(p.second);
            if (checkBest) {
                const std::vector<Scored> host = best_subset(fav[a], ro.mutationSeparation);
                bool same = host.size() == best.size();
                for (size_t i = 0; same && i < host.size(); ++i)
                    same = host[i].code == best[i].code && host[i].score == best[i].score;
                if (!same) throw DeviceError("k_best_subset differs from the host BestSubset");
            }
            std::vector<Mutation> muts;
            for (const Scored& s : best) muts.push_back(mutation_from_code(s.code));
            if (best.size() > 1) {
                std::string next;
                std::vector<int> mtp;
                if (apply_mutations(zmws_[zi].tpl, muts, &next, &mtp) && history[k].count(next)) {
                    best.resize(1);
                    muts.resize(1);
                }
            }
            (*nApplied)[k] += (long long)best.size();
            history[k].insert(zmws_[zi].tpl);
            centers[k].clear();
            for (const Scored& s : fav[a]) centers[k].push_back(mut_pos(s.code));
            HZmw& z = zmws_[zi];
            std::vector<int> mtp;
            if (!apply_host(&z.tpl, muts, &mtp)) {
                done[k] = 1;
                converged->at(k) = -1;
                if (retireDone) Retire({zi});
                continue;
            }
            UploadTemplate(zi);
            const bool last = zit[k] + 1 >= ro.maxIterations;
            const bool refill = !(last && retireDone);
            for (int q = 0; q < z.nReads; ++q) {
                HRead& r = reads_[z.readBegin + q];
                r.ts = mtp[r.ts];
                r.te = mtp[r.te];
                if (r.active && refill) {
                    EnsureCapacity(z.readBegin + q);
                    changed.push_back(z.readBegin + q);
                }
            }
            if (!refill) Retire({zi});
            if (++zit[k] >= ro.maxIterations) done[k] = 1;
        }
        descDirty_ = true;
        if (!qvNow.empty()) {
            std::vector<std::vector<int>> q;
            QVs(qvNow, &q);
            for (size_t i = 0; i < qvNow.size(); ++i) (*qvsOnConverge)[qvIdx[i]] = std::move(q[i]);
            if (reclaim_) Retire(qvNow);
        }
        const Clock::time_point t2 = Clock::now();
        if (!changed.empty()) {
            FillReads(changed);
            for (int r : changed)
                if (reads_[r].status != kFillOk) reads_[r].active = false;
            descDirty_ = true;
        }
        if (roundTrace) {
            const Clock::time_point t3 = Clock::now();
            std::fprintf(stderr, "[round] batch=%p round=%d zmws=%zu muts=%lld refill=%zu prerefill=%zu replayed=%lld "
                                 "score=%.1fms select=%.1fms fill=%.1fms bandtop=%.2fGB\n",
                         (void*)this, round, act.size(), rTotalMut_, changed.size(), preRefill.size(), replayed,
                         ms(t0, t1), ms(t1, t2), ms(t2, t3), valTop_ * 8.0 / 1e9);
        }
    }
    if (!finalRefill.empty()) {
        FillReads(finalRefill);
        for (int r : finalRefill)
            if (reads_[r].status != kFillOk) reads_[r].active = false;
        descDirty_ = true;
    }
}

void ArrowBatch::QVs(const std::vector<int>& zl, std::vector<std::vector<int>>* qvs)
{
    const StreamScope bound(stream_);
    RunRound(zl, nullptr, -std::numeric_limits<double>::max(), true);
    std::vector<long long> qvBase(zl.size());
    for (size_t k = 0; k < zl.size(); ++k) qvBase[k] = rPosStart_[k];
    upload(dWQvBase_, qvBase, stream_);
    dQv_.reserve(std::max<long long>(rTotalPos_, 1), false);
    ScoreWork W;
    W.nWork = (int)zl.size();
    W.zmw = dWZmw_.ptr;
    W.nMut = dWNMut_.ptr;
    W.mutBase = dWMutBase_.ptr;
    W.deltaBase = dWDeltaBase_.ptr;
    W.waveStart = dWWaveStart_.ptr;
    W.mutStart = dWMutStart_.ptr;
    W.posStart = dWPosStart_.ptr;
    W.codes = dCodes_.ptr;
    W.delta = dDelta_.ptr;
    const DevBatch B = View();
    Timed(kKQv, [&] {
        launch_qv(B, W, rTotalPos_, dWPosBase_.ptr, dPosOff_.ptr, dScore_.ptr, dWQvBase_.ptr, dQv_.ptr, stream_);
    });
    PBCCS_HIP(hipGetLastError());
    std::vector<int> q;
    download(q, dQv_, rTotalPos_, stream_);
    PBCCS_HIP(hipStreamSynchronize(stream_));
    qvs->assign(zl.size(), {});
    for (size_t k = 0; k < zl.size(); ++k) (*qvs)[k].assign(q.begin() + rPosStart_[k], q.begin() + rPosStart_[k + 1]);
}

}
```

pbccs_amd/csrc/fill_coop.hip:

```cpp
#include "arrow_device.hpp"
#include "arrow_kernels.hpp"
#include "coop_chain.hpp"

#include <algorithm>
#include <cstdlib>
#include <stdexcept>

namespace pbccs {
namespace {

using namespace coop;

template <int G>
struct Task {
    Group<G> g;
    int I, J, L, start;
    const unsigned* rdW;
    const unsigned* tpW;
    const double* ctx;
    double* lds0;
    double* lds1;
    double* glob0;
    double* glob1;
    int hcap;
    int rowsCap;
    bool gcol;
    int ckK;
    bool chainExit;
    int slackDiv;
    double prNot, prThird, sdn;
    double sdnInvLow;
    double sdnInvHigh;
    double devScale;
    double sdnInv;
    int r;
    double* pool;
    unsigned long long* bump;
    long long limit;
    long long* gA;
    long long* gB;
    long long* gCap;

    bool split;
    __device__ __forceinline__ int lrow(int k) const { return split ? (k & 1) * (hcap >> 1) + (k >> 1) : k; }
    __device__ __forceinline__ double* cptr(int b, int k) const
    {
        if (!gcol) return lds0 + (b ? hcap : 0) + lrow(k);
        return k < hcap ? lds0 + (b ? hcap : 0) + lrow(k) : glob0 + (b ? glob1 - glob0 : 0) + (k - hcap);
    }
    __device__ __forceinline__ double cget(int b, int k) const { return *cptr(b, k); }
    __device__ __forceinline__ void cset(int b, int k, double v) const { *cptr(b, k) = v; }
    __device__ __forceinline__ int TBase(int idx) const
    {
        return nib(tpW, max(idx, 0));
    }
    __device__ __forceinline__ int TCtx(int idx) const
    {
        return (start + idx + 1 < L) ? ctx_code(TBase(idx), TBase(idx + 1)) : kCtxZero;
    }
    __device__ __forceinline__ int RB(int x) const
    {
        return nib(rdW, x);
    }
};

struct PassOut {
    long long used;
    long long stored;
    double last;
    double sumL;
    bool tall;
    bool changed;
    bool regrow;
    int maxH;
    double dev;
    int unc;
};

struct Work {
    bool on;
    long long steps;
    long long issues;
};
__device__ __forceinline__ void count_issue(Work& W)
{
    if (W.on) {
        const unsigned long long act = __ballot(1);
        if ((int)(threadIdx.x & 63) == __ffsll((long long)act) - 1) W.issues += 1;
    }
}

__device__ __forceinline__ void col_fence(bool gcol)
{
    if (gcol) __builtin_amdgcn_fence(__ATOMIC_ACQ_REL, "workgroup");
}

__device__ __forceinline__ bool thr_ge(double x, double pm, double lo, double hi, bool& amb)
{
    const bool ge = x >= pm * hi;
    const bool lt = x < pm * lo;
    amb = pm != 0.0 && (pm < 0x1p-960 || (!ge && !lt));
    return ge || pm == 0.0;
}

__device__ __forceinline__ double scan_col_dev(double D, int chunks, int rowsPerChunk)
{
    return D + (4.0 * (double)chunks * (double)rowsPerChunk + 40.0 * (double)chunks + 8.0) * kUnitRoundoff;
}
__device__ __forceinline__ bool near_thr(double x, double t, double margin)
{
    const double mx = fmax(x, t);
    return mx > 0.0 && fabs(x - t) <= margin * mx;
}

template <int G>
__device__ __forceinline__ void copy_vals(int lane, double* __restrict__ dst, const double* __restrict__ src, long long n)
{
    long long k = lane;
    for (; k + 3 * G < n; k += 4 * G) {
        const double x0 = src[k], x1 = src[k + G], x2 = src[k + 2 * G], x3 = src[k + 3 * G];
        dst[k] = x0;
        dst[k + G] = x1;
        dst[k + 2 * G] = x2;
        dst[k + 3 * G] = x3;
    }
    for (; k < n; k += G) dst[k] = src[k];
}

template <int G>
__device__ bool regrow_bands(const Task<G>& T, Band& m, Band& o, bool mIsAlpha, long long need, long long keepO)
{
    if (!T.bump) return false;
    const long long full = (long long)(T.I + 1) * (T.J + 1) + 1;
    long long cap = max(need, keepO);
    cap = max(min(cap + cap / T.slackDiv + 64, full), max(need, keepO));
    unsigned long long base = 0;
    if (T.g.lane == 0) base = atomicAdd(T.bump, (unsigned long long)(2 * cap));
    base = (unsigned long long)__shfl((long long)base, 0, G);
    if (base + 2 * (unsigned long long)cap > (unsigned long long)T.limit) return false;
    __threadfence();
    double* na = T.pool + base;
    double* nb = na + cap;
    double* nm = mIsAlpha ? na : nb;
    double* no = mIsAlpha ? nb : na;
    copy_vals<G>(T.g.lane, no, o.val, keepO);
    m.val = nm;
    o.val = no;
    m.cap = cap;
    o.cap = cap;
    if (T.g.lane == 0) {
        T.gA[T.r] = (long long)base;
        T.gB[T.r] = (long long)base + cap;
        T.gCap[T.r] = cap;
    }
    return true;
}

template <int G>
__device__ double finish_log_scales(const Task<G>& T, const Band& m, int J)
{
    __builtin_amdgcn_fence(__ATOMIC_ACQ_REL, "workgroup");
    double s = 0.0;
    if (T.g.lane == 0) {
        int k = 0;
        for (; k + 7 <= J; k += 8) {
            double v[8];
#pragma unroll
            for (int q = 0; q < 8; ++q) v[q] = m.L(k + q);
#pragma unroll
            for (int q = 0; q < 8; ++q) s = s + v[q];
        }
        for (; k <= J; ++k) s = s + m.L(k);
    }
    return T.g.bcast(s, 0);
}

#ifndef PBCCS_TALL_PREFETCH
#define PBCCS_TALL_PREFETCH 1
#endif
template <int G, int R, bool SCAN, bool GC>
__device__ PassOut coop_alpha(const Task<G>& T, Band& a, Band& o, bool guided, bool selfValid, bool& ovf, long long keepO,
                              Work& W)
{
    constexpr int CH = G * R;
    constexpr bool PF = GC || (G == 64 && PBCCS_TALL_PREFETCH && !SCAN);
    constexpr bool PFS = GC || (G == 64 && PBCCS_TALL_PREFETCH);
    const Band* guide = guided ? &o : nullptr;
    const int I = T.I, J = T.J, lane = T.g.lane;
    PassOut out{0, 0, 0.0, 0.0, false, !selfValid, false, 1, 0.0, 0};
    bool counting = false;
    (void)keepO;
    if (a.cap < 1) ovf = true;
    if (lane == 0) {
        if (!ovf) a.V(0) = 1.0;
        a.R(0) = make_int2(0, 1);
        a.O(0) = 0;
        a.L(0) = 0.0;
    }
    int prev = 0, cur = 1;
    if (lane == 0) T.cset(prev, 0, 1.0);
    int pb = 0, pe = 1;
    double D = 0.0;
    int unc = 0;
    long long used = 1, stored = 1;
    int hb = 1, he = 1;
    int prevCtx = kCtxZero;
    int curBase = T.TBase(0), curCtx = T.TCtx(0);
    int tA = T.TBase(1), tB = T.TBase(2);
    double myF = 1.0;
    int2 gR = make_int2(0, 0), sR = make_int2(0, 0), gN = make_int2(0, 0), sN = make_int2(0, 0);
    {
        const int jj = G == 64 ? 1 + lane : 1;
        if (guide && jj < J) gN = guide->R(jj);
        if (selfValid && jj < J) sN = a.R(jj);
    }
    for (int j = 1; j < J; ++j) {
        const int jb = (j - 1) & (G - 1);
        int gx = 0, gy = 0, sx = 0, sy = 0;
        if constexpr (G == 64) {
            if (jb == 0) {
                gR = gN;
                sR = sN;
                const int jj = j + G + lane;
                if (guide && jj < J) gN = guide->R(jj);
                if (selfValid && jj < J) sN = a.R(jj);
            }
            if (guide) { gx = T.g.bcast(gR.x, jb); gy = T.g.bcast(gR.y, jb); }
            if (selfValid) { sx = T.g.bcast(sR.x, jb); sy = T.g.bcast(sR.y, jb); }
        } else {
            gR = gN;
            sR = sN;
            if (guide && j + 1 < J) gN = guide->R(j + 1);
            if (selfValid && j + 1 < J) sN = a.R(j + 1);
            gx = gR.x; gy = gR.y; sx = sR.x; sy = sR.y;
        }
        (void)jb;
        if (guide) {
            if (gx < gy) { hb = min(gx, hb); he = max(gy, he); }
        }
        if (selfValid) {
            if (sx < sy) { hb = min(sx, hb); he = max(sy, he); }
        }
        const int reqEnd = min(I, he);
        const int nextBase = tA, nextCtx = (T.start + j + 1 < T.L) ? ctx_code(tA, tB) : kCtxZero;
        const int tC = T.TBase(j + 2);
        const double* cp = T.ctx + curCtx * kCtxStride;
        const double* pp = T.ctx + prevCtx * kCtxStride;
        const double pMatch = pp[kM], pDel = pp[kD];
        const double cBranch = cp[kB], cStick3 = cp[kS3];
        const int b = hb;
        double mx = 0.0, aLast[R];
        int e = b, nc = 0;
        if (b < I) {
            double carry = 0.0;
            auto load_prev = [&](int ibx, double (&dst)[R + 1]) {
#pragma unroll
                for (int q = 0; q <= R; ++q) {
                    const int row = ibx - 1 + q;
                    dst[q] = (row >= pb && row < pe) ? T.cget(prev, row - pb) : 0.0;
                }
            };
            double pvN[R + 1];
            if constexpr (PF) load_prev(b + lane * R, pvN);
            for (int i0 = b;; i0 += CH) {
                if ((nc + 1) * CH > T.rowsCap) {
                    out.tall = true;
                    out.used = used;
                    W.steps += nc;
                    return out;
                }
                count_issue(W);
                const int ib = i0 + lane * R;
                double m[R], k[R], d[R], x[R];
                {
                    double pv[R + 1];
                    if constexpr (PF) {
#pragma unroll
                        for (int q = 0; q <= R; ++q) pv[q] = pvN[q];
                        load_prev(ib + CH, pvN);
                    } else {
                        load_prev(ib, pv);
                    }
#pragma unroll
                    for (int r = 0; r < R; ++r) {
                        const int i = ib + r;
                        const int rb = (i >= 1 && i <= I) ? T.RB(i - 1) : 15;
                        const double mpe = pv[r] * (rb == curBase ? T.prNot : T.prThird);
                        m[r] = (i == 1 && j == 1) ? mpe : ((i != 1 && j != 1) ? mpe * pMatch : 0.0);
                        k[r] = (i > 1) ? (rb == nextBase ? cBranch : cStick3) : 0.0;
                        d[r] = (j > 1) ? pv[r + 1] * pDel : 0.0;
                        x[r] = 0.0;
                    }
                }
                bool nz = false;
#pragma unroll
                for (int r = 0; r < R; ++r) nz = nz || m[r] != 0.0 || d[r] != 0.0;
                const unsigned long long nzb = T.g.bits(nz);
                if (carry != 0.0 || nzb != 0) {
                    const int startLane = ((G == 64 || R > 1) && carry == 0.0) ? __ffsll((long long)nzb) - 1 : 0;
                    if constexpr (R == 1) {
                        const int i = ib;
                        if (G == 64 && T.chainExit) {
                            auto maybe_stop = [&](double xv) {
                                const double pmv = fmax(mx, prefix_max<G>(xv));
                                return T.g.bits((i + 1 >= I) || (xv < pmv * T.sdnInvLow && i + 1 >= reqEnd));
                            };
                            x[0] = insertion_chain64_exit(m[0], k[0], d[0], carry, min(reqEnd, I) - 1 - i0, maybe_stop,
                                                          startLane);
                        } else {
                            x[0] = insertion_chain<G>(m[0], k[0], d[0], carry);
                        }
                    } else {
                        auto maybe_stop = [&](const double (&xv)[R]) {
                            double lp = xv[0];
#pragma unroll
                            for (int r = 1; r < R; ++r) lp = fmax(lp, xv[r]);
                            const double ex = shift_up<G>(prefix_max<G>(lp), 0.0);
                            double run = fmax(mx, ex);
                            bool st = false;
#pragma unroll
                            for (int r = 0; r < R; ++r) {
                                run = fmax(run, xv[r]);
                                const int i = ib + r;
                                st = st || (i + 1 >= I) || (xv[r] < run * T.sdnInvLow && i + 1 >= reqEnd);
                            }
                            return T.g.bits(st);
                        };
                        const int firstRow = min(reqEnd, I) - 1 - i0;
                        if constexpr (SCAN) {
                            scan_chain64<R>(m, k, d, carry, x);
                        } else {
                            insertion_chain_rows<G, R>(m, k, d, carry, x, firstRow < 0 ? 0 : firstRow / R, T.chainExit,
                                                       startLane, maybe_stop);
                        }
                    }
                }
                double pmR[R];
                if constexpr (R == 1) {
                    pmR[0] = fmax(mx, prefix_max<G>(x[0]));
                } else {
                    double lp = x[0];
#pragma unroll
                    for (int r = 1; r < R; ++r) lp = fmax(lp, x[r]);
                    double run = fmax(mx, shift_up<G>(prefix_max<G>(lp), 0.0));
#pragma unroll
                    for (int r = 0; r < R; ++r) {
                        run = fmax(run, x[r]);
                        pmR[r] = run;
                    }
                }
                bool ge[R], amb = false;
#pragma unroll
                for (int r = 0; r < R; ++r) {
                    const int i = ib + r;
                    bool a;
                    ge[r] = thr_ge(x[r], pmR[r], T.sdnInvLow, T.sdnInvHigh, a);
                    amb = amb || (a && i + 1 < I && i + 1 >= reqEnd);
                }
                if (__ballot(amb) != 0) {
#pragma unroll
                    for (int r = 0; r < R; ++r) ge[r] = x[r] >= pmR[r] / T.sdn;
                }
                int fs = R;
#pragma unroll
                for (int r = R - 1; r >= 0; --r) {
                    const int i = ib + r;
                    const bool cont = (i + 1 < I) && (ge[r] || i + 1 < reqEnd);
                    if (!cont) fs = r;
                }
                const unsigned long long stop = T.g.bits(fs < R);
                const int lastLane = stop ? (__ffsll((long long)stop) - 1) : (G - 1);
                double pmAt = pmR[R - 1];
#pragma unroll
                for (int r = 0; r < R - 1; ++r)
                    if (r == fs) pmAt = pmR[r];
                if (SCAN && i0 + CH >= reqEnd) {
                    const double mg = T.devScale * (2.0 * scan_col_dev(D, nc + 1, CH) + 8.0 * kUnitRoundoff);
                    const int rsStop = stop ? T.g.bcast(fs, lastLane) : R;
                    bool u = false;
#pragma unroll
                    for (int r = 0; r < R; ++r) {
                        const int i = ib + r;
                        const bool matters = (i + 1 < I) && (i + 1 >= reqEnd);
                        const bool upto = !stop || lane < lastLane || (lane == lastLane && r <= rsStop);
                        u = u || (matters && upto && near_thr(x[r], pmR[r] * T.sdnInv, mg));
                    }
                    if (T.g.bits(u) != 0) unc |= 1;
                }
                mx = T.g.bcast(pmAt, lastLane);
                ++nc;
                if (stop) {
                    const int rs = R == 1 ? 0 : T.g.bcast(fs, lastLane);
                    e = i0 + lastLane * R + rs + 1;
#pragma unroll
                    for (int r = 0; r < R; ++r) aLast[r] = x[r];
                    break;
                }
#pragma unroll
                for (int r = 0; r < R; ++r) T.cset(cur, (nc - 1) * CH + lane * R + r, x[r]);
                carry = T.g.bcast_last(x[R - 1]);
            }
        }
        const bool keep = T.ckK == 0 || ckpt_col_a(j, J, T.ckK);
        const long long add = keep ? e - b : 0;
        if (!ovf && !counting && stored + add + 1 > a.cap) {
            if (T.bump) counting = true;
            else ovf = true;
        }
        const bool store = !ovf && !counting && keep;
        const double thrF = mx / T.sdn;
        const bool scale = (mx != 0.0 && mx != 1.0);
        int nhb = e;
        bool found = false;
        const double mh = SCAN ? T.devScale * (3.0 * scan_col_dev(D, nc, CH) + 4.0 * kUnitRoundoff) : 0.0;
        auto load_cur = [&](int cx, double (&dst)[R]) {
#pragma unroll
            for (int r = 0; r < R; ++r) dst[r] = (cx == nc - 1) ? aLast[r] : T.cget(cur, cx * CH + lane * R + r);
        };
        double xN[R];
        if constexpr (PFS) load_cur(0, xN);
#pragma unroll 2
        for (int c = 0; c < nc; ++c) {
            int fh = R;
            double vv[R];
            double xc[R];
            if constexpr (PFS) {
#pragma unroll
                for (int r = 0; r < R; ++r) xc[r] = xN[r];
                if (c + 1 < nc) load_cur(c + 1, xN);
            } else {
                load_cur(c, xc);
            }
#pragma unroll
            for (int r = 0; r < R; ++r) {
                const int kk = c * CH + lane * R + r;
                const bool ok = b + kk < e;
                const double x = xc[r];
                const double v = scale ? x / mx : x;
                if (ok) {
                    T.cset(cur, kk, v);
                    if (store && stored + kk < a.cap) a.V(stored + kk) = v;
                }
                if (fh == R && ok && !(v < thrF)) fh = r;
                vv[r] = ok ? v : -1.0;
            }
            const unsigned long long hit = T.g.bits(fh < R);
            if constexpr (SCAN) {
                if (!found) {
                    const int hl = hit ? __ffsll((long long)hit) - 1 : G;
                    const int fhl = hit ? T.g.bcast(fh, hl) : R;
                    bool u = false;
#pragma unroll
                    for (int r = 0; r < R; ++r)
                        u = u || (vv[r] >= 0.0 && (lane < hl || (lane == hl && r <= fhl)) && near_thr(vv[r], thrF, mh));
                    if (T.g.bits(u) != 0) unc |= 2;
                }
            }
            if (!found && hit) {
                const int hl = __ffsll((long long)hit) - 1;
                nhb = b + c * CH + hl * R + (R == 1 ? 0 : T.g.bcast(fh, hl));
                found = true;
            }
        }
        if constexpr (SCAN) D = scan_col_dev(D, nc, CH) + kUnitRoundoff;
        if (!counting && stored + add > a.cap) ovf = true;
        out.changed = out.changed || b != sx || e != sy;
        out.maxH = max(out.maxH, e - b);
        if (lane == 0 && !counting) {
            a.R(j) = make_int2(b, e);
            a.O(j) = (int)stored;
        }
        if (lane == jb) myF = scale ? mx : 1.0;
        if ((jb == G - 1 || j == J - 1) && !counting && lane <= jb) a.L(j - jb + lane) = (myF != 1.0) ? log(myF) : 0.0;
        used += e - b;
        stored += add;
        W.steps += nc;
        col_fence(T.gcol && nc * CH > T.hcap);
        prev ^= 1;
        cur ^= 1;
        pb = b;
        pe = e;
        prevCtx = curCtx;
        curBase = nextBase;
        curCtx = nextCtx;
        tA = tB;
        tB = tC;
        he = e;
        hb = nhb;
    }
    const double em = (T.RB(I - 1) == T.TBase(J - 1)) ? T.prNot : T.prThird;
    const bool lastIn = I - 1 >= pb && I - 1 < pe;
    const double lik = (lastIn ? T.cget(prev, I - 1 - pb) : 0.0) * em;
    const double c = (0.0 < lik) ? lik : 0.0;
    double v = lik, ls = 0.0;
    if (c != 0.0 && c != 1.0) { v = lik / c; ls = log(c); }
    if (!ovf && !counting && stored + 1 > a.cap) {
        if (T.bump) counting = true;
        else ovf = true;
    }
    out.regrow = counting;
    if (lane == 0 && !counting) {
        if (!ovf) a.V(stored) = v;
        a.R(J) = make_int2(I, I + 1);
        a.O(J) = (int)stored;
        a.L(J) = ls;
    }
    out.used = used + 1;
    out.stored = stored + 1;
    out.last = v;
    if (!counting) out.sumL = finish_log_scales<G>(T, a, J);
    if constexpr (SCAN) {
        out.dev = T.devScale * (1.01 * (D + 4.0 * kUnitRoundoff) +
                                2.0 * (double)(J + 4) * kUnitRoundoff * (fabs(out.sumL) + fabs(log(fmax(v, 1e-300))) + 64.0));
        out.unc = unc | ((lastIn && v == 0.0) ? 1 : 0);
    }
    return out;
}

template <int G, int R, bool SCAN, bool GC>
__device__ PassOut coop_beta(const Task<G>& T, Band& bm, Band& o, bool guided, bool selfValid, bool& ovf, long long keepO,
                             Work& W)
{
    constexpr int CH = G * R;
    constexpr bool PF = GC || (G == 64 && PBCCS_TALL_PREFETCH && !SCAN);
    constexpr bool PFS = GC || (G == 64 && PBCCS_TALL_PREFETCH);
    const Band* guide = guided ? &o : nullptr;
    const int I = T.I, J = T.J, lane = T.g.lane;
    PassOut out{0, 0, 0.0, 0.0, false, !selfValid, false, 1, 0.0, 0};
    bool counting = false;
    (void)keepO;
    if (bm.cap < 1) ovf = true;
    if (lane == 0) {
        if (!ovf) bm.V(0) = 1.0;
        bm.R(J) = make_int2(I, I + 1);
        bm.O(J) = 0;
        bm.L(J) = 0.0;
    }
    int nxt = 0, cur = 1;
    if (lane == 0) T.cset(nxt, 0, 1.0);
    int pb = I, pe = I + 1;
    double D = 0.0;
    int unc = 0;
    long long used = 1, stored = 1;
    int hb = I, he = I;
    int nextBase = T.TBase(J - 1);
    int tA = T.TBase(J - 2), tB = nextBase;
    double myF = 1.0;
    int2 gR = make_int2(0, 0), sR = make_int2(0, 0), gN = make_int2(0, 0), sN = make_int2(0, 0);
    {
        const int jj = G == 64 ? J - 1 - lane : J - 1;
        if (guide && jj > 0) gN = guide->R(jj);
        if (selfValid && jj > 0) sN = bm.R(jj);
    }
    for (int j = J - 1; j > 0; --j) {
        const int jb = (J - 1 - j) & (G - 1);
        int gx = 0, gy = 0, sx = 0, sy = 0;
        if constexpr (G == 64) {
            if (jb == 0) {
                gR = gN;
                sR = sN;
                const int jj = j - G - lane;
                if (guide && jj > 0) gN = guide->R(jj);
                if (selfValid && jj > 0) sN = bm.R(jj);
            }
            if (guide) { gx = T.g.bcast(gR.x, jb); gy = T.g.bcast(gR.y, jb); }
            if (selfValid) { sx = T.g.bcast(sR.x, jb); sy = T.g.bcast(sR.y, jb); }
        } else {
            gR = gN;
            sR = sN;
            if (guide && j - 1 > 0) gN = guide->R(j - 1);
            if (selfValid && j - 1 > 0) sN = bm.R(j - 1);
            gx = gR.x; gy = gR.y; sx = sR.x; sy = sR.y;
        }
        (void)jb;
        const int curBase = tA, curCtx = (T.start + j < T.L) ? ctx_code(tA, tB) : kCtxZero;
        const int tC = T.TBase(j - 2);
        if (guide) {
            if (gx < gy) { hb = min(gx, hb); he = max(gy, he); }
        }
        if (selfValid) {
            if (sx < sy) { hb = min(sx, hb); he = max(sy, he); }
        }
        const int reqBegin = max(0, hb);
        const double* cp = T.ctx + curCtx * kCtxStride;
        const double cMatch = cp[kM], cDel = cp[kD], cBranch = cp[kB], cStick3 = cp[kS3];
        const int e = he;
        double mx = 0.0, aLast[R];
        int b = e, nc = 0;
        if (e - 1 > 0) {
            double carry = 0.0;
            auto load_next = [&](int obx, double (&dst)[R + 1]) {
#pragma unroll
                for (int q = 0; q <= R; ++q) {
                    const int row = e - obx - q;
                    dst[q] = (row >= pb && row < pe) ? T.cget(nxt, pe - 1 - row) : 0.0;
                }
            };
            double pvN[R + 1];
            if constexpr (PF) load_next(lane * R, pvN);
            for (int c = 0;; ++c) {
                if ((c + 1) * CH > T.rowsCap) {
                    out.tall = true;
                    out.used = used;
                    W.steps += nc;
                    return out;
                }
                count_issue(W);
                const int ob = c * CH + lane * R;
                double m[R], k[R], d[R], x[R];
                {
                    double pv[R + 1];
                    if constexpr (PF) {
#pragma unroll
                        for (int q = 0; q <= R; ++q) pv[q] = pvN[q];
                        load_next(ob + CH, pvN);
                    } else {
                        load_next(ob, pv);
                    }
#pragma unroll
                    for (int r = 0; r < R; ++r) {
                        const int i = e - 1 - ob - r;
                        const int nb = (i >= 0 && i < I) ? T.RB(i) : 15;
                        const bool same = nb == nextBase;
                        const double mpe = pv[r] * (same ? T.prNot : T.prThird);
                        m[r] = (i < I - 1) ? mpe * cMatch : ((i == I - 1 && j == J - 1) ? mpe : 0.0);
                        k[r] = (i < I - 1 && i > 0) ? (same ? cBranch : cStick3) : 0.0;
                        d[r] = (j < J - 1 && j > 0) ? pv[r + 1] * cDel : 0.0;
                        x[r] = 0.0;
                    }
                }
                bool nz = false;
#pragma unroll
                for (int r = 0; r < R; ++r) nz = nz || m[r] != 0.0 || d[r] != 0.0;
                const unsigned long long nzb = T.g.bits(nz);
                if (carry != 0.0 || nzb != 0) {
                    const int startLane = ((G == 64 || R > 1) && carry == 0.0) ? __ffsll((long long)nzb) - 1 : 0;
                    if constexpr (R == 1) {
                        const int i = e - 1 - ob;
                        if (G == 64 && T.chainExit) {
                            auto maybe_stop = [&](double xv) {
                                const double pmv = fmax(mx, prefix_max<G>(xv));
                                return T.g.bits((i - 1 <= 0) || (xv < pmv * T.sdnInvLow && i - 1 < reqBegin));
                            };
                            x[0] = insertion_chain64_exit(m[0], k[0], d[0], carry, e - 1 - max(1, reqBegin) - c * G,
                                                          maybe_stop, startLane);
                        } else {
                            x[0] = insertion_chain<G>(m[0], k[0], d[0], carry);
                        }
                    } else {
                        auto maybe_stop = [&](const double (&xv)[R]) {
                            double lp = xv[0];
#pragma unroll
                            for (int r = 1; r < R; ++r) lp = fmax(lp, xv[r]);
                            const double ex = shift_up<G>(prefix_max<G>(lp), 0.0);
                            double run = fmax(mx, ex);
                            bool st = false;
#pragma unroll
                            for (int r = 0; r < R; ++r) {
                                run = fmax(run, xv[r]);
                                const int i = e - 1 - ob - r;
                                st = st || (i - 1 <= 0) || (xv[r] < run * T.sdnInvLow && i - 1 < reqBegin);
                            }
                            return T.g.bits(st);
                        };
                        const int firstOff = e - 1 - max(1, reqBegin) - c * CH;
                        if constexpr (SCAN) {
                            scan_chain64<R>(m, k, d, carry, x);
                        } else {
                            insertion_chain_rows<G, R>(m, k, d, carry, x, firstOff < 0 ? 0 : firstOff / R, T.chainExit,
                                                       startLane, maybe_stop);
                        }
                    }
                }
                double pmR[R];
                if constexpr (R == 1) {
                    pmR[0] = fmax(mx, prefix_max<G>(x[0]));
                } else {
                    double lp = x[0];
#pragma unroll
                    for (int r = 1; r < R; ++r) lp = fmax(lp, x[r]);
                    double run = fmax(mx, shift_up<G>(prefix_max<G>(lp), 0.0));
#pragma unroll
                    for (int r = 0; r < R; ++r) {
                        run = fmax(run, x[r]);
                        pmR[r] = run;
                    }
                }
                bool ge[R], amb = false;
#pragma unroll
                for (int r = 0; r < R; ++r) {
                    const int i = e - 1 - ob - r;
                    bool a;
                    ge[r] = thr_ge(x[r], pmR[r], T.sdnInvLow, T.sdnInvHigh, a);
                    amb = amb || (a && i - 1 > 0 && i - 1 < reqBegin);
                }
                if (__ballot(amb) != 0) {
#pragma unroll
                    for (int r = 0; r < R; ++r) ge[r] = x[r] >= pmR[r] / T.sdn;
                }
                int fs = R;
#pragma unroll
                for (int r = R - 1; r >= 0; --r) {
                    const int i = e - 1 - ob - r;
                    const bool cont = (i - 1 > 0) && (ge[r] || i - 1 >= reqBegin);
                    if (!cont) fs = r;
                }
                const unsigned long long stop = T.g.bits(fs < R);
                const int lastLane = stop ? (__ffsll((long long)stop) - 1) : (G - 1);
                double pmAt = pmR[R - 1];
#pragma unroll
                for (int r = 0; r < R - 1; ++r)
                    if (r == fs) pmAt = pmR[r];
                if (SCAN && e - (c + 1) * CH - 1 < reqBegin) {
                    const double mg = T.devScale * (2.0 * scan_col_dev(D, nc + 1, CH) + 8.0 * kUnitRoundoff);
                    const int rsStop = stop ? T.g.bcast(fs, lastLane) : R;
                    bool u = false;
#pragma unroll
                    for (int r = 0; r < R; ++r) {
                        const int i = e - 1 - ob - r;
                        const bool matters = (i - 1 > 0) && (i - 1 < reqBegin);
                        const bool upto = !stop || lane < lastLane || (lane == lastLane && r <= rsStop);
                        u = u || (matters && upto && near_thr(x[r], pmR[r] * T.sdnInv, mg));
                    }
                    if (T.g.bits(u) != 0) unc |= 1;
                }
                mx = T.g.bcast(pmAt, lastLane);
                ++nc;
                if (stop) {
                    const int rs = R == 1 ? 0 : T.g.bcast(fs, lastLane);
                    b = e - 1 - (c * CH + lastLane * R + rs);
#pragma unroll
                    for (int r = 0; r < R; ++r) aLast[r] = x[r];
                    break;
                }
#pragma unroll
                for (int r = 0; r < R; ++r) T.cset(cur, ob + r, x[r]);
                carry = T.g.bcast_last(x[R - 1]);
            }
        }
        const bool keep = T.ckK == 0 || ckpt_col_b(j, J, T.ckK);
        const long long add = keep ? e - b : 0;
        if (!ovf && !counting && stored + add + 1 > bm.cap) {
            if (T.bump) counting = true;
            else ovf = true;
        }
        const bool store = !ovf && !counting && keep;
        const double thrF = mx / T.sdn;
        const bool scale = (mx != 0.0 && mx != 1.0);
        int nhe = b;
        bool found = false;
        const double mh = SCAN ? T.devScale * (3.0 * scan_col_dev(D, nc, CH) + 4.0 * kUnitRoundoff) : 0.0;
        auto load_cur = [&](int cx, double (&dst)[R]) {
#pragma unroll
            for (int r = 0; r < R; ++r) dst[r] = (cx == nc - 1) ? aLast[r] : T.cget(cur, cx * CH + lane * R + r);
        };
        double xN[R];
        if constexpr (PFS) load_cur(0, xN);
#pragma unroll 2
        for (int c = 0; c < nc; ++c) {
            int fh = R;
            double vv[R];
            double xc[R];
            if constexpr (PFS) {
#pragma unroll
                for (int r = 0; r < R; ++r) xc[r] = xN[r];
                if (c + 1 < nc) load_cur(c + 1, xN);
            } else {
                load_cur(c, xc);
            }
#pragma unroll
            for (int r = 0; r < R; ++r) {
                const int off = c * CH + lane * R + r;
                const bool ok = e - 1 - off >= b;
                const double x = xc[r];
                const double v = scale ? x / mx : x;
                if (ok) {
                    T.cset(cur, off, v);
                    if (store && stored + off < bm.cap) bm.V(stored + off) = v;
                }
                if (fh == R && ok && !(v < thrF)) fh = r;
                vv[r] = ok ? v : -1.0;
            }
            const unsigned long long hit = T.g.bits(fh < R);
            if constexpr (SCAN) {
                if (!found) {
                    const int hl = hit ? __ffsll((long long)hit) - 1 : G;
                    const int fhl = hit ? T.g.bcast(fh, hl) : R;
                    bool u = false;
#pragma unroll
                    for (int r = 0; r < R; ++r)
                        u = u || (vv[r] >= 0.0 && (lane < hl || (lane == hl && r <= fhl)) && near_thr(vv[r], thrF, mh));
                    if (T.g.bits(u) != 0) unc |= 2;
                }
            }
            if (!found && hit) {
                const int hl = __ffsll((long long)hit) - 1;
                nhe = e - (c * CH + hl * R + (R == 1 ? 0 : T.g.bcast(fh, hl)));
                found = true;
            }
        }
        if constexpr (SCAN) D = scan_col_dev(D, nc, CH) + kUnitRoundoff;
        if (!counting && stored + add > bm.cap) ovf = true;
        out.changed = out.changed || b != sx || e != sy;
        out.maxH = max(out.maxH, e - b);
        if (lane == 0 && !counting) {
            bm.R(j) = make_int2(b, e);
            bm.O(j) = (int)stored;
        }
        if (lane == jb) myF = scale ? mx : 1.0;
        if ((jb == G - 1 || j == 1) && !counting && lane <= jb) bm.L(j + jb - lane) = (myF != 1.0) ? log(myF) : 0.0;
        used += e - b;
        stored += add;
        W.steps += nc;
        col_fence(T.gcol && nc * CH > T.hcap);
        nxt ^= 1;
        cur ^= 1;
        pb = b;
        pe = e;
        hb = b;
        he = nhe;
        nextBase = curBase;
        tB = tA;
        tA = tC;
    }
    const double em = (T.TBase(0) == T.RB(0)) ? T.prNot : T.prThird;
    const bool lastIn = 1 >= pb && 1 < pe;
    const double raw = em * (lastIn ? T.cget(nxt, pe - 2) : 0.0);
    const double c = (0.0 < raw) ? raw : 0.0;
    double v = raw, ls = 0.0;
    if (c != 0.0 && c != 1.0) { v = raw / c; ls = log(c); }
    if (!ovf && !counting && stored + 1 > bm.cap) {
        if (T.bump) counting = true;
        else ovf = true;
    }
    out.regrow = counting;
    if (lane == 0 && !counting) {
        if (!ovf) bm.V(stored) = v;
        bm.R(0) = make_int2(0, 1);
        bm.O(0) = (int)stored;
        bm.L(0) = ls;
    }
    out.used = used + 1;
    out.stored = stored + 1;
    out.last = v;
    if (!counting) out.sumL = finish_log_scales<G>(T, bm, J);
    if constexpr (SCAN) {
        out.dev = T.devScale * (1.01 * (D + 4.0 * kUnitRoundoff) +
                                2.0 * (double)(J + 4) * kUnitRoundoff * (fabs(out.sumL) + fabs(log(fmax(v, 1e-300))) + 64.0));
        out.unc = unc | ((lastIn && v == 0.0) ? 1 : 0);
    }
    return out;
}

}

template <int G, bool GC, int R, bool SCAN>
__device__ __forceinline__ void fill_read(const DevBatch& B, const CoopFill& F, const int* __restrict__ reads, int n,
                                          int t, unsigned char* gbase)
{
    const int lane = threadIdx.x & (G - 1);
    double* col = reinterpret_cast<double*>(gbase);
    double* ctx = col + 2 * F.hcap;
    unsigned* rdW = reinterpret_cast<unsigned*>(ctx + kCtxDoubles + 1);
    unsigned* tpW = rdW + F.readWords;

    const bool valid = t < n;
    if (F.trace && valid && lane == 0) {
        F.trace[6LL * t] = (long long)wall_clock64();
        F.trace[6LL * t + 2] = (long long)clock64();
    }
    int r = 0, z = 0, I = 0, J = 0;
    TplView tv{};
    bool bad = true;
    if (valid) {
        r = reads[t];
        z = B.rZmw[r];
        I = B.rLen[r];
        tv = window_view(B, r);
        J = tv.Length();
        bad = I < 1 || J < 1 || (I + 7) / 8 > F.readWords || (J + 8) / 8 > F.tplWords;
        if (!bad) {
            const double* zc = B.zCtx + (long long)z * kCtxDoubles;
            for (int k = lane; k < kCtxDoubles; k += G) ctx[k] = zc[k];
        }
        if (!bad) {
            const char* rd = B.seqPool + B.rSeqOff[r];
            for (int w = lane; w < (I + 7) / 8; w += G) {
                unsigned word = 0;
                for (int q = 0; q < 8; ++q) {
                    const int x = 8 * w + q;
                    word |= (unsigned)(x < I ? base_code(rd[x]) : kBaseOther) << (4 * q);
                }
                rdW[w] = word;
            }
            for (int w = lane; w < (J + 8) / 8; w += G) {
                unsigned word = 0;
                for (int q = 0; q < 8; ++q) {
                    const int x = 8 * w + q;
                    const int g = tv.start + x;
                    word |= (unsigned)((x <= J && g < tv.L) ? base_code(tv.T[g]) : kBaseOther) << (4 * q);
                }
                tpW[w] = word;
            }
        }
    }
    __builtin_amdgcn_fence(__ATOMIC_ACQ_REL, "workgroup");
    if (!valid) return;
    if (bad) {
        if (lane == 0) B.rStatus[r] = (I < 1 || J < 1) ? kFillBadInput : kFillOverflow;
        return;
    }

    Task<G> T;
    T.g.lane = lane;
    T.g.base = (int)threadIdx.x & ~(G - 1);
    T.I = I;
    T.J = J;
    T.L = tv.L;
    T.start = tv.start;
    T.rdW = rdW;
    T.tpW = tpW;
    T.ctx = ctx;
    T.lds0 = col;
    T.lds1 = col + F.hcap;
    T.glob0 = GC ? F.colScratch + (size_t)t * 2 * F.gRows : nullptr;
    T.glob1 = GC ? T.glob0 + F.gRows : nullptr;
    T.hcap = F.hcap;
    T.split = R == 2;
    T.rowsCap = GC ? F.hcap + F.gRows : F.hcap;
    T.gcol = GC;
    T.chainExit = F.chainExit;
    T.ckK = B.rCkpt ? B.rCkpt[r] : 0;
    T.slackDiv = max(1, F.regrowSlackDiv);
    T.prNot = B.prNot;
    T.prThird = B.prThird;
    T.sdn = B.sdn;
    T.sdnInvLow = (1.0 / B.sdn) * (1.0 - F.thrMargin);
    T.sdnInvHigh = (1.0 / B.sdn) * (1.0 + F.thrMargin);
    T.devScale = F.devScale;
    T.sdnInv = 1.0 / B.sdn;
    T.r = r;
    T.pool = B.valPool;
    T.bump = F.valBump;
    T.limit = F.valLimit;
    T.gA = F.rValA;
    T.gB = F.rValB;
    T.gCap = F.rValCap;

    const long long cb = B.rColBase[r];
    Band a, bm;
    a.range = B.aRange + cb;
    a.off = B.aOff + cb;
    a.ls = B.aLs + cb;
    a.val = B.valPool + B.rValA[r];
    a.cap = B.rValCap[r];
    bm.range = B.bRange + cb;
    bm.off = B.bOff + cb;
    bm.ls = B.bLs + cb;
    bm.val = B.valPool + B.rValB[r];
    bm.cap = B.rValCap[r];

    bool ovf = false;
    long long needA = 0, needB = 0;
    unsigned long long cells = 0, passes = 0;
    int flips = 0;
    Work W{F.work != nullptr, 0, 0};
    unsigned long long regrowCells = 0, abortCells = 0;
    bool tallAbort = false;
    PassOut pa{0, 0, 0.0, 0.0, false, false, false, 0, 0.0, 0}, pb{0, 0, 0.0, 0.0, false, false, false, 0, 0.0, 0};
    int maxH = 0;
    long long ua = 0, ub = 0;
    long long sa = 0, sb = 0;
    const int maxSize = (int)(0.5 + kRebandFrac * (I + 1) * (J + 1));
    bool mismatched = false;
    int uncAny = 0;
    int unchanged = 0;
    int regrows = 0;
    for (int step = 0;; ++step) {
        bool doAlpha;
        if (step < 2) doAlpha = step == 0;
        else if (step == 2 && !(ua >= maxSize || ub >= maxSize)) {
            step = 5;
            doAlpha = true;
        } else doAlpha = step == 2 || step == 4;
        if (step == 5) {
            if (flips == 0 || flips == 3) {
                const double la = log(pa.last) + pa.sumL, lb = log(pb.last) + pb.sumL;
                mismatched = fabs(la - lb) > kAlphaBetaTol;
                if constexpr (SCAN)
                    if (isfinite(la) && isfinite(lb) &&
                        fabs(fabs(la - lb) - kAlphaBetaTol) <= pa.dev + pb.dev + 8.0 * kUnitRoundoff * fmax(fabs(la), fabs(lb)))
                        uncAny |= 4;
            }
        }
        if (step >= 5) {
            if (!(mismatched && flips <= kMaxFlipFlops)) break;
            doAlpha = flips % 2 == 0;
        }
        const bool guided = step > 0, self = step > 1;
        PassOut o;
        if (doAlpha) o = coop_alpha<G, R, SCAN, GC>(T, a, bm, guided, self, ovf, ub, W);
        else o = coop_beta<G, R, SCAN, GC>(T, bm, a, guided, self, ovf, ua, W);
        uncAny |= o.unc;
        if (o.tall) {
            tallAbort = true;
            abortCells = cells + (unsigned long long)o.used;
            break;
        }
        if (o.regrow) {
            regrowCells += (unsigned long long)o.used;
            const bool moved = ++regrows <= 8 && (doAlpha ? regrow_bands<G>(T, a, bm, true, o.stored, sb)
                                                          : regrow_bands<G>(T, bm, a, false, o.stored, sa));
            if (!moved) ovf = true;
            --step;
            continue;
        }
        cells += o.used;
        passes += 1;
        maxH = max(maxH, o.maxH);
        if (doAlpha) {
            pa = o;
            ua = o.used;
            sa = o.stored;
            needA = max(needA, o.stored);
        } else {
            pb = o;
            ub = o.used;
            sb = o.stored;
            needB = max(needB, o.stored);
        }
        if (step >= 2 && step <= 4) ++flips;
        if (step >= 5) {
            ++flips;
            unchanged = o.changed ? 0 : unchanged + 1;
            if (unchanged >= 2) {
                flips = kMaxFlipFlops + 1;
                break;
            }
        }
    }
    if (W.on) {
        unsigned long long* w = F.work + (G == 64 ? kFillWorkSlots : 0);
        if (W.issues) atomicAdd(&w[kFillWorkIssues], (unsigned long long)W.issues);
        if (lane == 0) {
            atomicAdd(&w[kFillWorkSteps], (unsigned long long)W.steps);
            atomicAdd(&w[kFillWorkReads], 1ull);
            atomicAdd(&w[kFillWorkRegrow], regrowCells);
            if (tallAbort) atomicAdd(&w[kFillWorkTallAbort], abortCells);
            else {
                atomicAdd(&w[ovf ? kFillWorkOverflow : kFillWorkCells], cells);
                if (!ovf) atomicAdd(&w[kFillWorkPasses], passes);
            }
        }
    }
    if (tallAbort) {
        if (lane == 0) B.rStatus[r] = kFillTall;
        return;
    }
    const double av = log(pa.last) + pa.sumL;
    const double bv = log(pb.last) + pb.sumL;
    const double mism = fabs(1.0 - av / bv);
    if constexpr (SCAN)
        if (isfinite(av) && isfinite(bv) && isfinite(mism) &&
            fabs(mism - kAlphaBetaTol) <= (pa.dev + fabs(av / bv) * pb.dev) / fabs(bv) + 8.0 * kUnitRoundoff)
            uncAny |= 8;
    if (lane == 0) {
        if (ovf) {
            B.rStatus[r] = kFillOverflow;
            F.usedA[r] = (int)needA;
            F.usedB[r] = (int)needB;
        } else if (SCAN && uncAny) {
            B.rStatus[r] = kFillUncertain;
            B.rFlips[r] = uncAny;
        } else {
            B.rFlips[r] = flips;
            B.rBaseline[r] = bv;
            B.rDev[r] = SCAN ? fmax(pa.dev, pb.dev) : 0.0;
            F.usedA[r] = (int)sa;
            F.usedB[r] = (int)sb;
            if (F.maxH) F.maxH[r] = maxH;
            B.rStatus[r] = (mism > kAlphaBetaTol) ? kFillMismatch : kFillOk;
            if (F.trace) {
                long long* tr = F.trace + 6LL * t;
                tr[1] = (long long)wall_clock64();
                tr[2] = (long long)clock64() - tr[2];
                tr[3] = (long long)cells;
                tr[4] = (long long)passes;
                tr[5] = (long long)J;
            }
            if (B.stats) {
                constexpr int kind = G == 64 ? kStatFillTall : kStatFill;
                atomicAdd(&B.stats[2 * kind], cells);
                atomicAdd(&B.stats[2 * kind + 1], 8ull * cells + 16ull * passes * (unsigned long long)(J + 1));
                atomicAdd(&B.stats[G == 64 ? 9 : 8], cells);
            }
        }
    }
}


template <int G, int MINW, bool GC, int R, bool SCAN>
__global__ void __launch_bounds__(64, MINW) k_fill_coop(DevBatch B, CoopFill F, const int* __restrict__ reads, int n)
{
    extern __shared__ __align__(16) unsigned char smem[];
    const long long wt0 = wave_t0(B.stats);
    if (F.prio) __builtin_amdgcn_s_setprio(3);
    const int grp = threadIdx.x / G;
    unsigned char* gbase = smem + (size_t)grp * F.groupBytes;
    fill_read<G, GC, R, SCAN>(B, F, reads, n, blockIdx.x * (64 / G) + grp, gbase);
    wave_ticks(B.stats, G == 64 ? kWaveFillTall : kWaveFill, wt0);
}

size_t coop_group_bytes(int hcap, int readWords, int tplWords)
{
    size_t b = (size_t)(2 * hcap + kCtxDoubles + 1) * sizeof(double) + (size_t)(readWords + tplWords) * 4;
    return (b + 15) & ~(size_t)15;
}

#ifndef PBCCS_NARROW_MINW
#define PBCCS_NARROW_MINW 2
#endif
void launch_fill_coop(int G, const DevBatch& B, const CoopFill& F, const int* reads, int n, hipStream_t s)
{
    if (n <= 0) return;
    const int per = 64 / G;
    const size_t lds = (size_t)per * F.groupBytes;
    if (lds > 160 * 1024) throw std::runtime_error("fill block needs more than 160 KB of LDS");
    using K = void (*)(DevBatch, CoopFill, const int*, int);
    const bool gc = F.colScratch != nullptr;
    const int R = gc ? std::min(F.rows, 2) : F.rows;
    struct Entry {
        int g, r;
        bool gc, scan;
        K k;
        bool attr;
    };
    static Entry ks[] = {
        {16, 1, false, false, (K)k_fill_coop<16, PBCCS_NARROW_MINW, false, 1, false>, false},
        {64, 1, false, false, (K)k_fill_coop<64, 2, false, 1, false>, false},
        {64, 2, false, false, (K)k_fill_coop<64, 2, false, 2, false>, false},
        {64, 2, false, true, (K)k_fill_coop<64, 2, false, 2, true>, false},
        {64, 1, true, false, (K)k_fill_coop<64, 1, true, 1, false>, false},
        {64, 2, true, false, (K)k_fill_coop<64, 1, true, 2, false>, false},
        {64, 2, true, true, (K)k_fill_coop<64, 1, true, 2, true>, false}};
    const bool scan = F.scan && G == 64 && R == 2;
    Entry* e = nullptr;
    for (Entry& x : ks)
        if (x.g == G && x.r == R && x.gc == gc && x.scan == scan) e = &x;
    if (!e) throw std::runtime_error("no fill kernel for this group size / rows per lane / column buffer");
    if (R > 1 && ((gc ? (F.hcap + F.gRows) : F.hcap) % (G * R) != 0 || F.hcap % 2 != 0))
        throw std::runtime_error("fill column buffers must hold whole chunks of G x rows rows (and even LDS rows)");
    if (!e->attr) {
        (void)hipFuncSetAttribute((const void*)e->k, hipFuncAttributeMaxDynamicSharedMemorySize, 160 * 1024);
        e->attr = true;
    }
    const dim3 grid((n + per - 1) / per);
    hipLaunchKernelGGL(e->k, grid, dim3(64), lds, s, B, F, reads, n);
}

}
```

Before: 3411.

## Spill cold fill state to LDS and split diagnostics into separate kernel

Moves per-read sequential state (pass results, band pointers, counters, regrow args) out of registers into a per-group LDS struct, and keeps cold regrow arguments in LDS for tall groups. Diagnostic counting and tracing become a compile-time template flag, with a separate diag kernel launched only when work or trace buffers are set. The goal is to cut VGPR/SGPR pressure in the hot fill kernels so they can reach higher occupancy or avoid spills. The cost is extra LDS per group, which may shrink the rows that fit, plus LDS round-trips for state accesses.

```diff
diff --git a/pbccs_amd/csrc/arrow_kernels.hpp b/pbccs_amd/csrc/arrow_kernels.hpp
--- a/pbccs_amd/csrc/arrow_kernels.hpp
+++ b/pbccs_amd/csrc/arrow_kernels.hpp
@@ -92,7 +92,7 @@
     kFillWorkCells = 0, kFillWorkTallAbort, kFillWorkRegrow, kFillWorkOverflow, kFillWorkSteps, kFillWorkIssues,
     kFillWorkReads, kFillWorkPasses, kFillWorkSlots
 };
-size_t coop_group_bytes(int hcap, int readWords, int tplWords);
+size_t coop_group_bytes(int G, int hcap, int readWords, int tplWords);
 constexpr int kNarrowGroupLanes = 16;
 constexpr int kTallRowsPerLane = 2;
 void launch_fill_coop(int G, const DevBatch& B, const CoopFill& F, const int* reads, int n, hipStream_t s);
diff --git a/pbccs_amd/csrc/engine.hip b/pbccs_amd/csrc/engine.hip
--- a/pbccs_amd/csrc/engine.hip
+++ b/pbccs_amd/csrc/engine.hip
@@ -964,9 +964,9 @@
     auto rows_for = [&](int p, int maxI, int w) -> int {
         if (p == 0) return 0;
         if (p == 1)
-            return (64 / narrowG) * coop_group_bytes(kCoopNarrowRows, w, 0) <= kCoopLdsBytes
+            return (64 / narrowG) * coop_group_bytes(narrowG, kCoopNarrowRows, w, 0) <= kCoopLdsBytes
                        ? kCoopNarrowRows : 0;
-        const long long room = (tallGroupLds - (long long)coop_group_bytes(0, w, 0)) / 16 / 64 * 64;
+        const long long room = (tallGroupLds - (long long)coop_group_bytes(tallG, 0, w, 0)) / 16 / 64 * 64;
         const long long full = full_rows(maxI);
         if (p == 2) {
             const long long want = std::min<long long>(kCoopTallRows, full);
@@ -974,7 +974,7 @@
         }
         static const long long hybLds = (long long)env_int("PBCCS_HYBRID_LDS_KB", (int)(kCoopLdsBytes >> 10)) << 10;
         static const long long hybRows = env_int("PBCCS_HYBRID_ROWS", kHybridRows);
-        const long long hroom = (std::min<long long>(hybLds, 160 << 10) - (long long)coop_group_bytes(0, w, 0)) / 16 / 64 * 64;
+        const long long hroom = (std::min<long long>(hybLds, 160 << 10) - (long long)coop_group_bytes(tallG, 0, w, 0)) / 16 / 64 * 64;
         const long long want = std::min(std::min(full, hroom), hybRows);
         return want >= 64 ? (int)want : 0;
     };
@@ -1095,7 +1095,7 @@
             F.prio = p >= 2;
             if (const char* e = std::getenv("PBCCS_FILL_THR_MARGIN"))
                 F.thrMargin = std::max(0x1p-50, std::atof(e));
-            F.groupBytes = coop_group_bytes(F.hcap, F.readWords, F.tplWords);
+            F.groupBytes = coop_group_bytes(G, F.hcap, F.readWords, F.tplWords);
             const int full = (int)full_rows(maxI);
             if (p == 3 && full > F.hcap) {
                 F.gRows = full - F.hcap;
diff --git a/pbccs_amd/csrc/fill_coop.hip b/pbccs_amd/csrc/fill_coop.hip
--- a/pbccs_amd/csrc/fill_coop.hip
+++ b/pbccs_amd/csrc/fill_coop.hip
@@ -10,59 +10,6 @@
 namespace {
 
 using namespace coop;
-
-template <int G>
-struct Task {
-    Group<G> g;
-    int I, J, L, start;
-    const unsigned* rdW;
-    const unsigned* tpW;
-    const double* ctx;
-    double* lds0;
-    double* lds1;
-    double* glob0;
-    double* glob1;
-    int hcap;
-    int rowsCap;
-    bool gcol;
-    int ckK;
-    bool chainExit;
-    int slackDiv;
-    double prNot, prThird, sdn;
-    double sdnInvLow;
-    double sdnInvHigh;
-    double devScale;
-    double sdnInv;
-    int r;
-    double* pool;
-    unsigned long long* bump;
-    long long limit;
-    long long* gA;
-    long long* gB;
-    long long* gCap;
-
-    bool split;
-    __device__ __forceinline__ int lrow(int k) const { return split ? (k & 1) * (hcap >> 1) + (k >> 1) : k; }
-    __device__ __forceinline__ double* cptr(int b, int k) const
-    {
-        if (!gcol) return lds0 + (b ? hcap : 0) + lrow(k);
-        return k < hcap ? lds0 + (b ? hcap : 0) + lrow(k) : glob0 + (b ? glob1 - glob0 : 0) + (k - hcap);
-    }
-    __device__ __forceinline__ double cget(int b, int k) const { return *cptr(b, k); }
-    __device__ __forceinline__ void cset(int b, int k, double v) const { *cptr(b, k) = v; }
-    __device__ __forceinline__ int TBase(int idx) const
-    {
-        return nib(tpW, max(idx, 0));
-    }
-    __device__ __forceinline__ int TCtx(int idx) const
-    {
-        return (start + idx + 1 < L) ? ctx_code(TBase(idx), TBase(idx + 1)) : kCtxZero;
-    }
-    __device__ __forceinline__ int RB(int x) const
-    {
-        return nib(rdW, x);
-    }
-};
 
 struct PassOut {
     long long used;
@@ -77,14 +24,124 @@
     int unc;
 };
 
+
+struct ColdArgs {
+    double* pool;
+    unsigned long long* bump;
+    long long limit;
+    long long* gA;
+    long long* gB;
+    long long* gCap;
+    int slackDiv;
+};
+struct PassKept {
+    long long used, stored;
+    double last, sumL, dev;
+};
+struct SeqState {
+    PassKept pa, pb;
+    double* valA;
+    double* valB;
+    long long cap;
+    long long used;
+    long long needA, needB;
+    unsigned long long cells, passes;
+    int flips, maxH, unchanged, regrows;
+    int uncAny;
+    int mismatched;
+    int r;
+    int ckK;
+};
+template <int G>
+struct FillState : SeqState {
+};
+template <>
+struct FillState<64> : SeqState {
+    ColdArgs cold;
+};
+template <int G>
+constexpr size_t state_bytes()
+{
+    return (sizeof(FillState<G>) + 15) & ~(size_t)15;
+}
+__device__ __forceinline__ void pass_fence() { asm volatile("" ::: "memory"); }
+
+template <int G>
+struct Task {
+    Group<G> g;
+    int I, J;
+    int tail;
+    const unsigned* rdW;
+    const unsigned* tpW;
+    const double* ctx;
+    double* lds0;
+    double* glob0;
+    double* glob1;
+    int hcap;
+    int rowsCap;
+    bool gcol;
+    bool chainExit;
+    double prNot, prThird, sdn;
+    double sdnInvLow;
+    double sdnInvHigh;
+    double sdnInv;
+    FillState<G>* st;
+    ColdArgs coldR;
+    __device__ __forceinline__ ColdArgs cold() const
+    {
+        if constexpr (G == 64) return st->cold;
+        else return coldR;
+    }
+    double devScale;
+    int ckKR;
+    __device__ __forceinline__ int ckK() const
+    {
+        if constexpr (G == 64) return ckKR;
+        else return st->ckK;
+    }
+    __device__ __forceinline__ void used_set(long long& reg, long long v) const
+    {
+        if constexpr (G == 64) reg = v;
+        else st->used = v;
+    }
+    __device__ __forceinline__ long long used_get(const long long& reg) const
+    {
+        if constexpr (G == 64) return reg;
+        else return st->used;
+    }
+
+    bool split;
+    __device__ __forceinline__ int lrow(int k) const { return split ? (k & 1) * (hcap >> 1) + (k >> 1) : k; }
+    __device__ __forceinline__ double* cptr(int b, int k) const
+    {
+        if (!gcol) return lds0 + (b ? hcap : 0) + lrow(k);
+        return k < hcap ? lds0 + (b ? hcap : 0) + lrow(k) : glob0 + (b ? glob1 - glob0 : 0) + (k - hcap);
+    }
+    __device__ __forceinline__ double cget(int b, int k) const { return *cptr(b, k); }
+    __device__ __forceinline__ void cset(int b, int k, double v) const { *cptr(b, k) = v; }
+    __device__ __forceinline__ int TBase(int idx) const
+    {
+        return nib(tpW, max(idx, 0));
+    }
+    __device__ __forceinline__ int TCtx(int idx) const
+    {
+        return (idx + 1 < tail) ? ctx_code(TBase(idx), TBase(idx + 1)) : kCtxZero;
+    }
+    __device__ __forceinline__ int RB(int x) const
+    {
+        return nib(rdW, x);
+    }
+};
+
 struct Work {
     bool on;
     long long steps;
     long long issues;
 };
+template <bool DIAG>
 __device__ __forceinline__ void count_issue(Work& W)
 {
-    if (W.on) {
+    if (DIAG && W.on) {
         const unsigned long long act = __ballot(1);
         if ((int)(threadIdx.x & 63) == __ffsll((long long)act) - 1) W.issues += 1;
     }
@@ -128,30 +185,30 @@
 }
 
 template <int G>
-__device__ bool regrow_bands(const Task<G>& T, Band& m, Band& o, bool mIsAlpha, long long need, long long keepO)
-{
-    if (!T.bump) return false;
+__device__ bool regrow_bands(const Task<G>& T, bool mIsAlpha, long long need, long long keepO)
+{
+    const ColdArgs C = T.cold();
+    SeqState& S = *T.st;
+    const int r = S.r;
+    if (!C.bump) return false;
     const long long full = (long long)(T.I + 1) * (T.J + 1) + 1;
     long long cap = max(need, keepO);
-    cap = max(min(cap + cap / T.slackDiv + 64, full), max(need, keepO));
+    cap = max(min(cap + cap / C.slackDiv + 64, full), max(need, keepO));
     unsigned long long base = 0;
-    if (T.g.lane == 0) base = atomicAdd(T.bump, (unsigned long long)(2 * cap));
+    if (T.g.lane == 0) base = atomicAdd(C.bump, (unsigned long long)(2 * cap));
     base = (unsigned long long)__shfl((long long)base, 0, G);
-    if (base + 2 * (unsigned long long)cap > (unsigned long long)T.limit) return false;
+    if (base + 2 * (unsigned long long)cap > (unsigned long long)C.limit) return false;
     __threadfence();
-    double* na = T.pool + base;
+    double* na = C.pool + base;
     double* nb = na + cap;
-    double* nm = mIsAlpha ? na : nb;
-    double* no = mIsAlpha ? nb : na;
-    copy_vals<G>(T.g.lane, no, o.val, keepO);
-    m.val = nm;
-    o.val = no;
-    m.cap = cap;
-    o.cap = cap;
+    copy_vals<G>(T.g.lane, mIsAlpha ? nb : na, mIsAlpha ? S.valB : S.valA, keepO);
+    S.valA = na;
+    S.valB = nb;
+    S.cap = cap;
     if (T.g.lane == 0) {
-        T.gA[T.r] = (long long)base;
-        T.gB[T.r] = (long long)base + cap;
-        T.gCap[T.r] = cap;
+        C.gA[r] = (long long)base;
+        C.gB[r] = (long long)base + cap;
+        C.gCap[r] = cap;
     }
     return true;
 }
@@ -178,7 +235,7 @@
 #ifndef PBCCS_TALL_PREFETCH
 #define PBCCS_TALL_PREFETCH 1
 #endif
-template <int G, int R, bool SCAN, bool GC>
+template <int G, int R, bool SCAN, bool GC, bool DIAG>
 __device__ PassOut coop_alpha(const Task<G>& T, Band& a, Band& o, bool guided, bool selfValid, bool& ovf, long long keepO,
                               Work& W)
 {
@@ -202,7 +259,9 @@
     int pb = 0, pe = 1;
     double D = 0.0;
     int unc = 0;
-    long long used = 1, stored = 1;
+    long long stored = 1;
+    long long usedR = 0;
+    T.used_set(usedR, 1);
     int hb = 1, he = 1;
     int prevCtx = kCtxZero;
     int curBase = T.TBase(0), curCtx = T.TCtx(0);
@@ -242,7 +301,7 @@
             if (sx < sy) { hb = min(sx, hb); he = max(sy, he); }
         }
         const int reqEnd = min(I, he);
-        const int nextBase = tA, nextCtx = (T.start + j + 1 < T.L) ? ctx_code(tA, tB) : kCtxZero;
+        const int nextBase = tA, nextCtx = (j + 1 < T.tail) ? ctx_code(tA, tB) : kCtxZero;
         const int tC = T.TBase(j + 2);
         const double* cp = T.ctx + curCtx * kCtxStride;
         const double* pp = T.ctx + prevCtx * kCtxStride;
@@ -265,11 +324,11 @@
             for (int i0 = b;; i0 += CH) {
                 if ((nc + 1) * CH > T.rowsCap) {
                     out.tall = true;
-                    out.used = used;
-                    W.steps += nc;
+                    out.used = T.used_get(usedR);
+                    if constexpr (DIAG) W.steps += nc;
                     return out;
                 }
-                count_issue(W);
+                count_issue<DIAG>(W);
                 const int ib = i0 + lane * R;
                 double m[R], k[R], d[R], x[R];
                 {
@@ -401,10 +460,11 @@
                 carry = T.g.bcast_last(x[R - 1]);
             }
         }
-        const bool keep = T.ckK == 0 || ckpt_col_a(j, J, T.ckK);
+        const int ckK = T.ckK();
+        const bool keep = ckK == 0 || ckpt_col_a(j, J, ckK);
         const long long add = keep ? e - b : 0;
         if (!ovf && !counting && stored + add + 1 > a.cap) {
-            if (T.bump) counting = true;
+            if (T.cold().bump) counting = true;
             else ovf = true;
         }
         const bool store = !ovf && !counting && keep;
@@ -472,9 +532,9 @@
         }
         if (lane == jb) myF = scale ? mx : 1.0;
         if ((jb == G - 1 || j == J - 1) && !counting && lane <= jb) a.L(j - jb + lane) = (myF != 1.0) ? log(myF) : 0.0;
-        used += e - b;
+        T.used_set(usedR, T.used_get(usedR) + (e - b));
         stored += add;
-        W.steps += nc;
+        if constexpr (DIAG) W.steps += nc;
         col_fence(T.gcol && nc * CH > T.hcap);
         prev ^= 1;
         cur ^= 1;
@@ -495,7 +555,7 @@
     double v = lik, ls = 0.0;
     if (c != 0.0 && c != 1.0) { v = lik / c; ls = log(c); }
     if (!ovf && !counting && stored + 1 > a.cap) {
-        if (T.bump) counting = true;
+        if (T.cold().bump) counting = true;
         else ovf = true;
     }
     out.regrow = counting;
@@ -505,7 +565,7 @@
         a.O(J) = (int)stored;
         a.L(J) = ls;
     }
-    out.used = used + 1;
+    out.used = T.used_get(usedR) + 1;
     out.stored = stored + 1;
     out.last = v;
     if (!counting) out.sumL = finish_log_scales<G>(T, a, J);
@@ -517,7 +577,7 @@
     return out;
 }
 
-template <int G, int R, bool SCAN, bool GC>
+template <int G, int R, bool SCAN, bool GC, bool DIAG>
 __device__ PassOut coop_beta(const Task<G>& T, Band& bm, Band& o, bool guided, bool selfValid, bool& ovf, long long keepO,
                              Work& W)
 {
@@ -541,7 +601,9 @@
     int pb = I, pe = I + 1;
     double D = 0.0;
     int unc = 0;
-    long long used = 1, stored = 1;
+    long long stored = 1;
+    long long usedR = 0;
+    T.used_set(usedR, 1);
     int hb = I, he = I;
     int nextBase = T.TBase(J - 1);
     int tA = T.TBase(J - 2), tB = nextBase;
@@ -573,7 +635,7 @@
             gx = gR.x; gy = gR.y; sx = sR.x; sy = sR.y;
         }
         (void)jb;
-        const int curBase = tA, curCtx = (T.start + j < T.L) ? ctx_code(tA, tB) : kCtxZero;
+        const int curBase = tA, curCtx = (j < T.tail) ? ctx_code(tA, tB) : kCtxZero;
         const int tC = T.TBase(j - 2);
         if (guide) {
             if (gx < gy) { hb = min(gx, hb); he = max(gy, he); }
@@ -601,11 +663,11 @@
             for (int c = 0;; ++c) {
                 if ((c + 1) * CH > T.rowsCap) {
                     out.tall = true;
-                    out.used = used;
-                    W.steps += nc;
+                    out.used = T.used_get(usedR);
+                    if constexpr (DIAG) W.steps += nc;
                     return out;
                 }
-                count_issue(W);
+                count_issue<DIAG>(W);
                 const int ob = c * CH + lane * R;
                 double m[R], k[R], d[R], x[R];
                 {
@@ -738,10 +800,11 @@
                 carry = T.g.bcast_last(x[R - 1]);
             }
         }
-        const bool keep = T.ckK == 0 || ckpt_col_b(j, J, T.ckK);
+        const int ckK = T.ckK();
+        const bool keep = ckK == 0 || ckpt_col_b(j, J, ckK);
         const long long add = keep ? e - b : 0;
         if (!ovf && !counting && stored + add + 1 > bm.cap) {
-            if (T.bump) counting = true;
+            if (T.cold().bump) counting = true;
             else ovf = true;
         }
         const bool store = !ovf && !counting && keep;
@@ -809,9 +872,9 @@
         }
         if (lane == jb) myF = scale ? mx : 1.0;
         if ((jb == G - 1 || j == 1) && !counting && lane <= jb) bm.L(j + jb - lane) = (myF != 1.0) ? log(myF) : 0.0;
-        used += e - b;
+        T.used_set(usedR, T.used_get(usedR) + (e - b));
         stored += add;
-        W.steps += nc;
+        if constexpr (DIAG) W.steps += nc;
         col_fence(T.gcol && nc * CH > T.hcap);
         nxt ^= 1;
         cur ^= 1;
@@ -830,7 +893,7 @@
     double v = raw, ls = 0.0;
     if (c != 0.0 && c != 1.0) { v = raw / c; ls = log(c); }
     if (!ovf && !counting && stored + 1 > bm.cap) {
-        if (T.bump) counting = true;
+        if (T.cold().bump) counting = true;
         else ovf = true;
     }
     out.regrow = counting;
@@ -840,7 +903,7 @@
         bm.O(0) = (int)stored;
         bm.L(0) = ls;
     }
-    out.used = used + 1;
+    out.used = T.used_get(usedR) + 1;
     out.stored = stored + 1;
     out.last = v;
     if (!counting) out.sumL = finish_log_scales<G>(T, bm, J);
@@ -854,18 +917,19 @@
 
 }
 
-template <int G, bool GC, int R, bool SCAN>
+template <int G, bool GC, int R, bool SCAN, bool DIAG>
 __device__ __forceinline__ void fill_read(const DevBatch& B, const CoopFill& F, const int* __restrict__ reads, int n,
                                           int t, unsigned char* gbase)
 {
     const int lane = threadIdx.x & (G - 1);
-    double* col = reinterpret_cast<double*>(gbase);
-    double* ctx = col + 2 * F.hcap;
-    unsigned* rdW = reinterpret_cast<unsigned*>(ctx + kCtxDoubles + 1);
+    double* ctx = reinterpret_cast<double*>(gbase);
+    FillState<G>& S = *reinterpret_cast<FillState<G>*>(ctx + kCtxDoubles + 1);
+    double* col = reinterpret_cast<double*>(reinterpret_cast<unsigned char*>(&S) + state_bytes<G>());
+    unsigned* rdW = reinterpret_cast<unsigned*>(col + 2 * F.hcap);
     unsigned* tpW = rdW + F.readWords;
 
     const bool valid = t < n;
-    if (F.trace && valid && lane == 0) {
+    if (DIAG && F.trace && valid && lane == 0) {
         F.trace[6LL * t] = (long long)wall_clock64();
         F.trace[6LL * t + 2] = (long long)clock64();
     }
@@ -916,13 +980,11 @@
     T.g.base = (int)threadIdx.x & ~(G - 1);
     T.I = I;
     T.J = J;
-    T.L = tv.L;
-    T.start = tv.start;
+    T.tail = tv.L - tv.start;
     T.rdW = rdW;
     T.tpW = tpW;
     T.ctx = ctx;
     T.lds0 = col;
-    T.lds1 = col + F.hcap;
     T.glob0 = GC ? F.colScratch + (size_t)t * 2 * F.gRows : nullptr;
     T.glob1 = GC ? T.glob0 + F.gRows : nullptr;
     T.hcap = F.hcap;
@@ -930,126 +992,147 @@
     T.rowsCap = GC ? F.hcap + F.gRows : F.hcap;
     T.gcol = GC;
     T.chainExit = F.chainExit;
-    T.ckK = B.rCkpt ? B.rCkpt[r] : 0;
-    T.slackDiv = max(1, F.regrowSlackDiv);
     T.prNot = B.prNot;
     T.prThird = B.prThird;
     T.sdn = B.sdn;
     T.sdnInvLow = (1.0 / B.sdn) * (1.0 - F.thrMargin);
     T.sdnInvHigh = (1.0 / B.sdn) * (1.0 + F.thrMargin);
+    T.sdnInv = 1.0 / B.sdn;
+    T.st = &S;
     T.devScale = F.devScale;
-    T.sdnInv = 1.0 / B.sdn;
-    T.r = r;
-    T.pool = B.valPool;
-    T.bump = F.valBump;
-    T.limit = F.valLimit;
-    T.gA = F.rValA;
-    T.gB = F.rValB;
-    T.gCap = F.rValCap;
-
-    const long long cb = B.rColBase[r];
-    Band a, bm;
-    a.range = B.aRange + cb;
-    a.off = B.aOff + cb;
-    a.ls = B.aLs + cb;
-    a.val = B.valPool + B.rValA[r];
-    a.cap = B.rValCap[r];
-    bm.range = B.bRange + cb;
-    bm.off = B.bOff + cb;
-    bm.ls = B.bLs + cb;
-    bm.val = B.valPool + B.rValB[r];
-    bm.cap = B.rValCap[r];
-
+    T.ckKR = B.rCkpt ? B.rCkpt[r] : 0;
+    {
+        ColdArgs C;
+        C.pool = B.valPool;
+        C.bump = F.valBump;
+        C.limit = F.valLimit;
+        C.gA = F.rValA;
+        C.gB = F.rValB;
+        C.gCap = F.rValCap;
+        C.slackDiv = max(1, F.regrowSlackDiv);
+        if constexpr (G == 64) S.cold = C;
+        else T.coldR = C;
+    }
+
+    S.pa = PassKept{0, 0, 0.0, 0.0, 0.0};
+    S.pb = PassKept{0, 0, 0.0, 0.0, 0.0};
+    S.valA = B.valPool + B.rValA[r];
+    S.valB = B.valPool + B.rValB[r];
+    S.cap = B.rValCap[r];
+    S.needA = 0;
+    S.needB = 0;
+    S.cells = 0;
+    S.passes = 0;
+    S.flips = 0;
+    S.maxH = 0;
+    S.unchanged = 0;
+    S.regrows = 0;
+    S.uncAny = 0;
+    S.mismatched = 0;
+    S.r = r;
+    S.ckK = T.ckKR;
     bool ovf = false;
-    long long needA = 0, needB = 0;
-    unsigned long long cells = 0, passes = 0;
-    int flips = 0;
-    Work W{F.work != nullptr, 0, 0};
+    Work W{DIAG && F.work != nullptr, 0, 0};
     unsigned long long regrowCells = 0, abortCells = 0;
     bool tallAbort = false;
-    PassOut pa{0, 0, 0.0, 0.0, false, false, false, 0, 0.0, 0}, pb{0, 0, 0.0, 0.0, false, false, false, 0, 0.0, 0};
-    int maxH = 0;
-    long long ua = 0, ub = 0;
-    long long sa = 0, sb = 0;
-    const int maxSize = (int)(0.5 + kRebandFrac * (I + 1) * (J + 1));
-    bool mismatched = false;
-    int uncAny = 0;
-    int unchanged = 0;
-    int regrows = 0;
     for (int step = 0;; ++step) {
         bool doAlpha;
         if (step < 2) doAlpha = step == 0;
-        else if (step == 2 && !(ua >= maxSize || ub >= maxSize)) {
-            step = 5;
+        else if (step == 2) {
+            const int maxSize = (int)(0.5 + kRebandFrac * (I + 1) * (J + 1));
+            if (!(S.pa.used >= maxSize || S.pb.used >= maxSize)) step = 5;
             doAlpha = true;
-        } else doAlpha = step == 2 || step == 4;
+        } else doAlpha = step == 4;
         if (step == 5) {
+            const int flips = S.flips;
             if (flips == 0 || flips == 3) {
-                const double la = log(pa.last) + pa.sumL, lb = log(pb.last) + pb.sumL;
-                mismatched = fabs(la - lb) > kAlphaBetaTol;
+                const double la = log(S.pa.last) + S.pa.sumL, lb = log(S.pb.last) + S.pb.sumL;
+                S.mismatched = fabs(la - lb) > kAlphaBetaTol;
                 if constexpr (SCAN)
                     if (isfinite(la) && isfinite(lb) &&
-                        fabs(fabs(la - lb) - kAlphaBetaTol) <= pa.dev + pb.dev + 8.0 * kUnitRoundoff * fmax(fabs(la), fabs(lb)))
-                        uncAny |= 4;
+                        fabs(fabs(la - lb) - kAlphaBetaTol) <=
+                            S.pa.dev + S.pb.dev + 8.0 * kUnitRoundoff * fmax(fabs(la), fabs(lb)))
+                        S.uncAny |= 4;
             }
         }
         if (step >= 5) {
-            if (!(mismatched && flips <= kMaxFlipFlops)) break;
+            const int flips = S.flips;
+            if (!(S.mismatched && flips <= kMaxFlipFlops)) break;
             doAlpha = flips % 2 == 0;
         }
         const bool guided = step > 0, self = step > 1;
+        pass_fence();
+        Band m, g;
+        {
+            const long long cb = B.rColBase[S.r];
+            m.range = (doAlpha ? B.aRange : B.bRange) + cb;
+            m.off = (doAlpha ? B.aOff : B.bOff) + cb;
+            m.ls = (doAlpha ? B.aLs : B.bLs) + cb;
+            m.val = doAlpha ? S.valA : S.valB;
+            m.cap = S.cap;
+            g.range = (doAlpha ? B.bRange : B.aRange) + cb;
+            g.off = nullptr;
+            g.ls = nullptr;
+            g.val = nullptr;
+            g.cap = 0;
+        }
         PassOut o;
-        if (doAlpha) o = coop_alpha<G, R, SCAN, GC>(T, a, bm, guided, self, ovf, ub, W);
-        else o = coop_beta<G, R, SCAN, GC>(T, bm, a, guided, self, ovf, ua, W);
-        uncAny |= o.unc;
+        if (doAlpha) o = coop_alpha<G, R, SCAN, GC, DIAG>(T, m, g, guided, self, ovf, 0, W);
+        else o = coop_beta<G, R, SCAN, GC, DIAG>(T, m, g, guided, self, ovf, 0, W);
+        pass_fence();
+        if constexpr (SCAN) S.uncAny |= o.unc;
         if (o.tall) {
             tallAbort = true;
-            abortCells = cells + (unsigned long long)o.used;
+            if constexpr (DIAG) abortCells = S.cells + (unsigned long long)o.used;
             break;
         }
         if (o.regrow) {
-            regrowCells += (unsigned long long)o.used;
-            const bool moved = ++regrows <= 8 && (doAlpha ? regrow_bands<G>(T, a, bm, true, o.stored, sb)
-                                                          : regrow_bands<G>(T, bm, a, false, o.stored, sa));
+            if constexpr (DIAG) regrowCells += (unsigned long long)o.used;
+            const int regrows = S.regrows + 1;
+            S.regrows = regrows;
+            const bool moved =
+                regrows <= 8 && regrow_bands<G>(T, doAlpha, o.stored, doAlpha ? S.pb.stored : S.pa.stored);
             if (!moved) ovf = true;
             --step;
             continue;
         }
-        cells += o.used;
-        passes += 1;
-        maxH = max(maxH, o.maxH);
+        S.cells += o.used;
+        S.passes += 1;
+        S.maxH = max(S.maxH, o.maxH);
+        const PassKept kept{o.used, o.stored, o.last, o.sumL, o.dev};
         if (doAlpha) {
-            pa = o;
-            ua = o.used;
-            sa = o.stored;
-            needA = max(needA, o.stored);
+            S.pa = kept;
+            S.needA = max(S.needA, o.stored);
         } else {
-            pb = o;
-            ub = o.used;
-            sb = o.stored;
-            needB = max(needB, o.stored);
-        }
-        if (step >= 2 && step <= 4) ++flips;
+            S.pb = kept;
+            S.needB = max(S.needB, o.stored);
+        }
+        if (step >= 2 && step <= 4) S.flips += 1;
         if (step >= 5) {
-            ++flips;
-            unchanged = o.changed ? 0 : unchanged + 1;
+            S.flips += 1;
+            const int unchanged = o.changed ? 0 : S.unchanged + 1;
+            S.unchanged = unchanged;
             if (unchanged >= 2) {
-                flips = kMaxFlipFlops + 1;
+                S.flips = kMaxFlipFlops + 1;
                 break;
             }
         }
     }
-    if (W.on) {
-        unsigned long long* w = F.work + (G == 64 ? kFillWorkSlots : 0);
-        if (W.issues) atomicAdd(&w[kFillWorkIssues], (unsigned long long)W.issues);
-        if (lane == 0) {
-            atomicAdd(&w[kFillWorkSteps], (unsigned long long)W.steps);
-            atomicAdd(&w[kFillWorkReads], 1ull);
-            atomicAdd(&w[kFillWorkRegrow], regrowCells);
-            if (tallAbort) atomicAdd(&w[kFillWorkTallAbort], abortCells);
-            else {
-                atomicAdd(&w[ovf ? kFillWorkOverflow : kFillWorkCells], cells);
-                if (!ovf) atomicAdd(&w[kFillWorkPasses], passes);
+    pass_fence();
+    const unsigned long long cells = S.cells, passes = S.passes;
+    if constexpr (DIAG) {
+        if (W.on) {
+            unsigned long long* w = F.work + (G == 64 ? kFillWorkSlots : 0);
+            if (W.issues) atomicAdd(&w[kFillWorkIssues], (unsigned long long)W.issues);
+            if (lane == 0) {
+                atomicAdd(&w[kFillWorkSteps], (unsigned long long)W.steps);
+                atomicAdd(&w[kFillWorkReads], 1ull);
+                atomicAdd(&w[kFillWorkRegrow], regrowCells);
+                if (tallAbort) atomicAdd(&w[kFillWorkTallAbort], abortCells);
+                else {
+                    atomicAdd(&w[ovf ? kFillWorkOverflow : kFillWorkCells], cells);
+                    if (!ovf) atomicAdd(&w[kFillWorkPasses], passes);
+                }
             }
         }
     }
@@ -1057,9 +1140,12 @@
         if (lane == 0) B.rStatus[r] = kFillTall;
         return;
     }
+    const PassKept pa = S.pa, pb = S.pb;
+    const int uncEnd = S.uncAny;
     const double av = log(pa.last) + pa.sumL;
     const double bv = log(pb.last) + pb.sumL;
     const double mism = fabs(1.0 - av / bv);
+    int uncAny = SCAN ? uncEnd : 0;
     if constexpr (SCAN)
         if (isfinite(av) && isfinite(bv) && isfinite(mism) &&
             fabs(mism - kAlphaBetaTol) <= (pa.dev + fabs(av / bv) * pb.dev) / fabs(bv) + 8.0 * kUnitRoundoff)
@@ -1067,26 +1153,28 @@
     if (lane == 0) {
         if (ovf) {
             B.rStatus[r] = kFillOverflow;
-            F.usedA[r] = (int)needA;
-            F.usedB[r] = (int)needB;
+            F.usedA[r] = (int)S.needA;
+            F.usedB[r] = (int)S.needB;
         } else if (SCAN && uncAny) {
             B.rStatus[r] = kFillUncertain;
             B.rFlips[r] = uncAny;
         } else {
-            B.rFlips[r] = flips;
+            B.rFlips[r] = S.flips;
             B.rBaseline[r] = bv;
             B.rDev[r] = SCAN ? fmax(pa.dev, pb.dev) : 0.0;
-            F.usedA[r] = (int)sa;
-            F.usedB[r] = (int)sb;
-            if (F.maxH) F.maxH[r] = maxH;
+            F.usedA[r] = (int)pa.stored;
+            F.usedB[r] = (int)pb.stored;
+            if (F.maxH) F.maxH[r] = S.maxH;
             B.rStatus[r] = (mism > kAlphaBetaTol) ? kFillMismatch : kFillOk;
-            if (F.trace) {
-                long long* tr = F.trace + 6LL * t;
-                tr[1] = (long long)wall_clock64();
-                tr[2] = (long long)clock64() - tr[2];
-                tr[3] = (long long)cells;
-                tr[4] = (long long)passes;
-                tr[5] = (long long)J;
+            if constexpr (DIAG) {
+                if (F.trace) {
+                    long long* tr = F.trace + 6LL * t;
+                    tr[1] = (long long)wall_clock64();
+                    tr[2] = (long long)clock64() - tr[2];
+                    tr[3] = (long long)cells;
+                    tr[4] = (long long)passes;
+                    tr[5] = (long long)J;
+                }
             }
             if (B.stats) {
                 constexpr int kind = G == 64 ? kStatFillTall : kStatFill;
@@ -1099,21 +1187,32 @@
 }
 
 
-template <int G, int MINW, bool GC, int R, bool SCAN>
-__global__ void __launch_bounds__(64, MINW) k_fill_coop(DevBatch B, CoopFill F, const int* __restrict__ reads, int n)
+template <int G, bool GC, int R, bool SCAN, bool DIAG>
+__device__ __forceinline__ void fill_block(const DevBatch& B, const CoopFill& F, const int* __restrict__ reads, int n)
 {
     extern __shared__ __align__(16) unsigned char smem[];
     const long long wt0 = wave_t0(B.stats);
     if (F.prio) __builtin_amdgcn_s_setprio(3);
     const int grp = threadIdx.x / G;
     unsigned char* gbase = smem + (size_t)grp * F.groupBytes;
-    fill_read<G, GC, R, SCAN>(B, F, reads, n, blockIdx.x * (64 / G) + grp, gbase);
+    fill_read<G, GC, R, SCAN, DIAG>(B, F, reads, n, blockIdx.x * (64 / G) + grp, gbase);
     wave_ticks(B.stats, G == 64 ? kWaveFillTall : kWaveFill, wt0);
 }
-
-size_t coop_group_bytes(int hcap, int readWords, int tplWords)
-{
-    size_t b = (size_t)(2 * hcap + kCtxDoubles + 1) * sizeof(double) + (size_t)(readWords + tplWords) * 4;
+template <int G, int MINW, bool GC, int R, bool SCAN>
+__global__ void __launch_bounds__(64, MINW) k_fill_coop(DevBatch B, CoopFill F, const int* __restrict__ reads, int n)
+{
+    fill_block<G, GC, R, SCAN, false>(B, F, reads, n);
+}
+template <int G, int MINW, bool GC, int R, bool SCAN>
+__global__ void __launch_bounds__(64, MINW) k_fill_coop_diag(DevBatch B, CoopFill F, const int* __restrict__ reads, int n)
+{
+    fill_block<G, GC, R, SCAN, true>(B, F, reads, n);
+}
+
+size_t coop_group_bytes(int G, int hcap, int readWords, int tplWords)
+{
+    const size_t st = G == 64 ? state_bytes<64>() : state_bytes<16>();
+    size_t b = (size_t)(2 * hcap + kCtxDoubles + 1) * sizeof(double) + st + (size_t)(readWords + tplWords) * 4;
     return (b + 15) & ~(size_t)15;
 }
 
@@ -1132,17 +1231,17 @@
     struct Entry {
         int g, r;
         bool gc, scan;
-        K k;
+        K k, diag;
         bool attr;
     };
     static Entry ks[] = {
-        {16, 1, false, false, (K)k_fill_coop<16, PBCCS_NARROW_MINW, false, 1, false>, false},
-        {64, 1, false, false, (K)k_fill_coop<64, 2, false, 1, false>, false},
-        {64, 2, false, false, (K)k_fill_coop<64, 2, false, 2, false>, false},
-        {64, 2, false, true, (K)k_fill_coop<64, 2, false, 2, true>, false},
-        {64, 1, true, false, (K)k_fill_coop<64, 1, true, 1, false>, false},
-        {64, 2, true, false, (K)k_fill_coop<64, 1, true, 2, false>, false},
-        {64, 2, true, true, (K)k_fill_coop<64, 1, true, 2, true>, false}};
+        {16, 1, false, false, (K)k_fill_coop<16, PBCCS_NARROW_MINW, false, 1, false>, (K)k_fill_coop_diag<16, 2, false, 1, false>, false},
+        {64, 1, false, false, (K)k_fill_coop<64, 2, false, 1, false>, (K)k_fill_coop_diag<64, 2, false, 1, false>, false},
+        {64, 2, false, false, (K)k_fill_coop<64, 2, false, 2, false>, (K)k_fill_coop_diag<64, 2, false, 2, false>, false},
+        {64, 2, false, true, (K)k_fill_coop<64, 2, false, 2, true>, (K)k_fill_coop_diag<64, 2, false, 2, true>, false},
+        {64, 1, true, false, (K)k_fill_coop<64, 1, true, 1, false>, (K)k_fill_coop_diag<64, 1, true, 1, false>, false},
+        {64, 2, true, false, (K)k_fill_coop<64, 1, true, 2, false>, (K)k_fill_coop_diag<64, 1, true, 2, false>, false},
+        {64, 2, true, true, (K)k_fill_coop<64, 1, true, 2, true>, (K)k_fill_coop_diag<64, 1, true, 2, true>, false}};
     const bool scan = F.scan && G == 64 && R == 2;
     Entry* e = nullptr;
     for (Entry& x : ks)
@@ -1152,10 +1251,12 @@
         throw std::runtime_error("fill column buffers must hold whole chunks of G x rows rows (and even LDS rows)");
     if (!e->attr) {
         (void)hipFuncSetAttribute((const void*)e->k, hipFuncAttributeMaxDynamicSharedMemorySize, 160 * 1024);
+        (void)hipFuncSetAttribute((const void*)e->diag, hipFuncAttributeMaxDynamicSharedMemorySize, 160 * 1024);
         e->attr = true;
     }
     const dim3 grid((n + per - 1) / per);
-    hipLaunchKernelGGL(e->k, grid, dim3(64), lds, s, B, F, reads, n);
-}
-
-}
+    const K k = (F.work || F.trace) ? e->diag : e->k;
+    hipLaunchKernelGGL(k, grid, dim3(64), lds, s, B, F, reads, n);
+}
+
+}
```

After: 3535 (median of 6 runs). +3.6%, better.
